# wing02/MyLdpcCppApi

Measured on AMD Instinct MI355X. Metric: decoded Mbit/s (info bits), DVB-S2 N=64800 rate-1/2, 50 iters, higher is better.
Workload: dtype f32; 1 GPU; DVB-S2-profile (64800,32400) rate-1/2 (seeded IRA table with the standard's structure, E=226799), batch 4096 frames per GPU, 50 iterations, sum-product fp32 (probability domain), all-zero codeword + AWGN sigma=0.95 (no frame converges), early termination on, inputs resident in HBM; global_batch=4096, frames_per_gpu=4096, algo=sp, frames_per_launch=4096, parallelism=frames sharded over 1 GPU(s), all-gather of decoded bytes, frames_converged=0

## Files before the change

### myldpccppapi_amd/csrc/flood_kernels.hpp

```cpp
#pragma once

#include <hip/hip_runtime.h>
#include <stdint.h>

#include "ldpc_expf.h"

namespace ldpc {

constexpr int kAlgoSP = 0;
constexpr int kAlgoMS = 1;
constexpr int kAlgoMSC = 2;
constexpr int kCompactCapacity = 512;
constexpr int kLastCapacity = 64;
constexpr int kBlock = 256;
constexpr int kWavesPerBlock = 4;
constexpr int kMaxUnrolledDegree = 16;
constexpr int kMaxUnrolledCheckDegreeMS = 32;

#ifndef LDPC_NT_LOAD
#define LDPC_NT_LOAD 1
#endif
#ifndef LDPC_NT_STORE
#define LDPC_NT_STORE 1
#endif
typedef float vf2 __attribute__((ext_vector_type(2)));
typedef float vf4 __attribute__((ext_vector_type(4)));

template <typename T> __device__ __forceinline__ T ld_stream(const T *p)
{
#if LDPC_NT_LOAD
    return __builtin_nontemporal_load(p);
#else
    return *p;
#endif
}
template <typename T> __device__ __forceinline__ void st_stream(T *p, T v)
{
#if LDPC_NT_STORE
    __builtin_nontemporal_store(v, p);
#else
    *p = v;
#endif
}

template <int V> __device__ __forceinline__ void vload(float (&d)[V], const float *p);
template <> __device__ __forceinline__ void vload<1>(float (&d)[1], const float *p) { d[0] = ld_stream(p); }
template <> __device__ __forceinline__ void vload<2>(float (&d)[2], const float *p)
{
    const vf2 t = ld_stream(reinterpret_cast<const vf2 *>(p));
    d[0] = t.x; d[1] = t.y;
}
template <> __device__ __forceinline__ void vload<4>(float (&d)[4], const float *p)
{
    const vf4 t = ld_stream(reinterpret_cast<const vf4 *>(p));
    d[0] = t.x; d[1] = t.y; d[2] = t.z; d[3] = t.w;
}
template <int V> __device__ __forceinline__ void vstore(float *p, const float (&s)[V]);
template <> __device__ __forceinline__ void vstore<1>(float *p, const float (&s)[1]) { st_stream(p, s[0]); }
template <> __device__ __forceinline__ void vstore<2>(float *p, const float (&s)[2])
{
    vf2 t; t.x = s[0]; t.y = s[1];
    st_stream(reinterpret_cast<vf2 *>(p), t);
}
template <> __device__ __forceinline__ void vstore<4>(float *p, const float (&s)[4])
{
    vf4 t; t.x = s[0]; t.y = s[1]; t.z = s[2]; t.w = s[3];
    st_stream(reinterpret_cast<vf4 *>(p), t);
}

typedef _Float16 hf;
typedef _Float16 vh2 __attribute__((ext_vector_type(2)));
typedef _Float16 vh4 __attribute__((ext_vector_type(4)));

template <int V> __device__ __forceinline__ void vload(float (&d)[V], const hf *p);
template <> __device__ __forceinline__ void vload<1>(float (&d)[1], const hf *p) { d[0] = (float)ld_stream(p); }
template <> __device__ __forceinline__ void vload<2>(float (&d)[2], const hf *p)
{
    const vh2 t = ld_stream(reinterpret_cast<const vh2 *>(p));
    d[0] = (float)t.x; d[1] = (float)t.y;
}
template <> __device__ __forceinline__ void vload<4>(float (&d)[4], const hf *p)
{
    const vh4 t = ld_stream(reinterpret_cast<const vh4 *>(p));
    d[0] = (float)t.x; d[1] = (float)t.y; d[2] = (float)t.z; d[3] = (float)t.w;
}
template <int V> __device__ __forceinline__ void vstore(hf *p, const float (&s)[V]);
template <> __device__ __forceinline__ void vstore<1>(hf *p, const float (&s)[1]) { st_stream(p, (hf)s[0]); }
template <> __device__ __forceinline__ void vstore<2>(hf *p, const float (&s)[2])
{
    vh2 t; t.x = (hf)s[0]; t.y = (hf)s[1];
    st_stream(reinterpret_cast<vh2 *>(p), t);
}
template <> __device__ __forceinline__ void vstore<4>(hf *p, const float (&s)[4])
{
    vh4 t; t.x = (hf)s[0]; t.y = (hf)s[1]; t.z = (hf)s[2]; t.w = (hf)s[3];
    st_stream(reinterpret_cast<vh4 *>(p), t);
}

__device__ __forceinline__ int wave_id_in_block()
{
    return __builtin_amdgcn_readfirstlane((int)(threadIdx.x >> 6));
}

template <int V> __device__ __forceinline__ bool tile_finished(const uint64_t *done, int tile)
{
    bool all = true;
#pragma unroll
    for (int v = 0; v < V; ++v) all = all && (done[(size_t)tile * V + v] == ~0ull);
    return all;
}

struct TailRef {
    const int32_t *state;
    int32_t base_tile;
    int32_t n_tiles;
};

template <int V> __device__ __forceinline__ int tile_select(const TailRef &t, const uint64_t *done, int row)
{
    int tile = row;
    if (t.state && __builtin_amdgcn_readfirstlane(t.state[0])) {
        if (row >= t.n_tiles) return -1;
        tile = t.base_tile + row;
    }
    return tile_finished<V>(done, tile) ? -1 : tile;
}


struct CheckArgs {
    const void *__restrict__ Q;
    void *__restrict__ R;
    const int32_t *__restrict__ cls_e0;
    const uint64_t *__restrict__ done;
    int64_t E;
    int32_t n_rows;
    int32_t rows_per_wave;
    int32_t degree;
    float ms_scale = 1.0f;
    TailRef tail;
    int32_t tiles_first = 0;
    float ms_offset = 0.0f;
    const void *__restrict__ first_chan = nullptr;
    const int32_t *__restrict__ edge_col = nullptr;
    int32_t N = 0;
    const int32_t *__restrict__ qpos = nullptr;
};

template <int D> __device__ __forceinline__ void row_slots(const int32_t *__restrict__ qpos, int e0, int lane, int (&slot)[D])
{
    static_assert(D <= 64, "one lane per edge");
    const int mine = qpos[e0 + (lane < D ? lane : D - 1)];
#pragma unroll
    for (int k = 0; k < D; ++k) slot[k] = __builtin_amdgcn_readlane(mine, k);
}
__device__ __forceinline__ int edge_slot(const int32_t *__restrict__ qpos, int e)
{
    return __builtin_amdgcn_readfirstlane(qpos[e]);
}

struct GridPos { int row, block; };
__device__ __forceinline__ GridPos grid_pos(int tiles_first)
{
    return tiles_first ? GridPos{(int)blockIdx.x, (int)blockIdx.y} : GridPos{(int)blockIdx.y, (int)blockIdx.x};
}

template <int D, int V>
__device__ __forceinline__ void check_sp(const float (&x)[D][V], float (&out)[D][V])
{
#pragma unroll
    for (int v = 0; v < V; ++v) {
        if (D == 1) { out[0][v] = 1.0f; continue; }
        {
            float p = x[1][v];
#pragma unroll
            for (int j = 2; j < D; ++j) p *= x[j][v];
            out[0][v] = p;
        }
        float pre = x[0][v];
#pragma unroll
        for (int k = 1; k < D; ++k) {
            float p = pre;
#pragma unroll
            for (int j = k + 1; j < D; ++j) p *= x[j][v];
            out[k][v] = p;
            pre *= x[k][v];
        }
    }
}

struct MsCorr {
    float scale, offset;
};
template <typename T> __device__ __forceinline__ float ms_corr(float m, const MsCorr &c)
{
    const float r = fmaxf(m - c.offset, 0.0f) * c.scale;
    return sizeof(T) == 2 ? (float)(hf)r : r;
}

template <int D, int V, bool CORR = false, typename T = float>
__device__ __forceinline__ void check_ms(const float (&x)[D][V], float (&out)[D][V], MsCorr c = MsCorr{1.0f, 0.0f})
{
#pragma unroll
    for (int v = 0; v < V; ++v) {
        float m1 = 1000.0f, m2 = 1000.0f;
        int idx = -1;
        unsigned par = 0;
#pragma unroll
        for (int j = 0; j < D; ++j) {
            const float a = __builtin_fabsf(x[j][v]);
            par ^= (x[j][v] < 0.0f) ? 1u : 0u;
            if (a < m1) { m2 = m1; m1 = a; idx = j; }
            else if (a < m2) { m2 = a; }
        }
        if (CORR) { m1 = ms_corr<T>(m1, c); m2 = ms_corr<T>(m2, c); }
#pragma unroll
        for (int k = 0; k < D; ++k) {
            const float b = (k == idx) ? m2 : m1;
            const unsigned s = par ^ ((x[k][v] < 0.0f) ? 1u : 0u);
            out[k][v] = s ? -b : b;
        }
    }
}

__device__ __forceinline__ MsCorr ms_corr_of(const CheckArgs &a) { return MsCorr{a.ms_scale, a.ms_offset}; }

template <int ALGO, int D, int V, int W, typename T>
__global__ __launch_bounds__(kBlock) void check_kernel(const CheckArgs a)
{
    constexpr size_t F = 64 * V;
    constexpr int SUB = V / W;
    const int lane = threadIdx.x & 63;
    const GridPos gp = grid_pos(a.tiles_first);
    const int tile = tile_select<V>(a.tail, a.done, gp.row);
    if (tile < 0) return;
    const int wave = gp.block * kWavesPerBlock + wave_id_in_block();
    const int sub = wave % SUB;
    const int r_begin = (wave / SUB) * a.rows_per_wave;
    const int r_end = min(r_begin + a.rows_per_wave, a.n_rows);
    const unsigned lane_off = (unsigned)sub * 64 * W + (unsigned)lane * W;
    const T *Qu = static_cast<const T *>(a.Q) + (size_t)tile * (size_t)a.E * F;
    T *Rt = static_cast<T *>(a.R) + (size_t)tile * (size_t)a.E * F + lane_off;

    const T *Ct = (ALGO != kAlgoSP && a.first_chan)
                      ? static_cast<const T *>(a.first_chan) + (size_t)tile * (size_t)a.N * F + lane_off : nullptr;
    for (int r = r_begin; r < r_end; ++r) {
        const int e0 = a.cls_e0[r];
        float x[D][W], out[D][W];
        if (ALGO != kAlgoSP && Ct) {
#pragma unroll
            for (int k = 0; k < D; ++k) vload<W>(x[k], Ct + (size_t)a.edge_col[e0 + k] * F);
        } else {
            int sl[D];
            row_slots<D>(a.qpos, e0, lane, sl);
#pragma unroll
            for (int k = 0; k < D; ++k) vload<W>(x[k], Qu + (size_t)sl[k] * F + lane_off);
        }
        if (ALGO == kAlgoSP) check_sp<D, W>(x, out); else if (ALGO == kAlgoMS) check_ms<D, W>(x, out); else check_ms<D, W, true, T>(x, out, ms_corr_of(a));
#pragma unroll
        for (int k = 0; k < D; ++k) vstore<W>(Rt + (size_t)(e0 + k) * F, out[k]);
    }
}

template <int ALGO, int V, typename T>
__device__ __forceinline__ void check_row_generic(const T *Qu, unsigned lane_off, T *Rt, int e0, int D,
                                                  const int32_t *__restrict__ qpos, const MsCorr &c)
{
    constexpr size_t F = 64 * V;
    if (ALGO != kAlgoSP) {
        float m1[V], m2[V];
        int idx[V];
        unsigned par[V];
#pragma unroll
        for (int v = 0; v < V; ++v) { m1[v] = 1000.0f; m2[v] = 1000.0f; idx[v] = -1; par[v] = 0; }
        for (int j = 0; j < D; ++j) {
            float xj[V];
            vload<V>(xj, Qu + (size_t)edge_slot(qpos, e0 + j) * F + lane_off);
#pragma unroll
            for (int v = 0; v < V; ++v) {
                const float m = __builtin_fabsf(xj[v]);
                par[v] ^= (xj[v] < 0.0f) ? 1u : 0u;
                if (m < m1[v]) { m2[v] = m1[v]; m1[v] = m; idx[v] = j; }
                else if (m < m2[v]) { m2[v] = m; }
            }
        }
        if (ALGO == kAlgoMSC) {
#pragma unroll
            for (int v = 0; v < V; ++v) { m1[v] = ms_corr<T>(m1[v], c); m2[v] = ms_corr<T>(m2[v], c); }
        }
        for (int k = 0; k < D; ++k) {
            float xk[V], o[V];
            vload<V>(xk, Qu + (size_t)edge_slot(qpos, e0 + k) * F + lane_off);
#pragma unroll
            for (int v = 0; v < V; ++v) {
                const float b = (k == idx[v]) ? m2[v] : m1[v];
                const unsigned sg = par[v] ^ ((xk[v] < 0.0f) ? 1u : 0u);
                o[v] = sg ? -b : b;
            }
            vstore<V>(Rt + (size_t)(e0 + k) * F, o);
        }
        return;
    }
    for (int k = 0; k < D; ++k) {
        float o[V];
        float p[V];
#pragma unroll
        for (int v = 0; v < V; ++v) p[v] = 1.0f;
        for (int j = 0; j < D; ++j) {
            if (j == k) continue;
            float xj[V];
            vload<V>(xj, Qu + (size_t)edge_slot(qpos, e0 + j) * F + lane_off);
#pragma unroll
            for (int v = 0; v < V; ++v) p[v] *= xj[v];
        }
#pragma unroll
        for (int v = 0; v < V; ++v) o[v] = p[v];
        vstore<V>(Rt + (size_t)(e0 + k) * F, o);
    }
}

template <int ALGO, int V, typename T>
__global__ __launch_bounds__(kBlock) void check_kernel_generic(const CheckArgs a)
{
    constexpr size_t F = 64 * V;
    const int lane = threadIdx.x & 63;
    const GridPos gp = grid_pos(a.tiles_first);
    const int tile = tile_select<V>(a.tail, a.done, gp.row);
    if (tile < 0) return;
    const int wave = gp.block * kWavesPerBlock + wave_id_in_block();
    const int r_begin = wave * a.rows_per_wave;
    const int r_end = min(r_begin + a.rows_per_wave, a.n_rows);
    const T *Qu = static_cast<const T *>(a.Q) + (size_t)tile * (size_t)a.E * F;
    T *Rt = static_cast<T *>(a.R) + (size_t)tile * (size_t)a.E * F + (size_t)lane * V;
    for (int r = r_begin; r < r_end; ++r) check_row_generic<ALGO, V, T>(Qu, (unsigned)lane * V, Rt, a.cls_e0[r], a.degree, a.qpos, ms_corr_of(a));
}

struct GroupClass {
    int32_t block_begin;
    int32_t degree;
    int32_t count;
    int32_t pad;
    const int32_t *ids;
    const int32_t *edges;
    int64_t q_base;
};

template <int ALGO, int D, int V, int W, typename T>
__device__ __forceinline__ void check_rows(const T *Qu, unsigned lane_off, T *Rt, const int32_t *__restrict__ e0s, int r_begin, int r_end,
                                           const T *Ct, const int32_t *__restrict__ edge_col,
                                           const int32_t *__restrict__ qpos, const MsCorr &c)
{
    const int lane = threadIdx.x & 63;
    constexpr size_t F = 64 * V;
    for (int r = r_begin; r < r_end; ++r) {
        const int e0 = e0s[r];
        float x[D][W], out[D][W];
        if (ALGO != kAlgoSP && Ct) {
#pragma unroll
            for (int k = 0; k < D; ++k) vload<W>(x[k], Ct + (size_t)edge_col[e0 + k] * F);
        } else {
            int sl[D];
            row_slots<D>(qpos, e0, lane, sl);
#pragma unroll
            for (int k = 0; k < D; ++k) vload<W>(x[k], Qu + (size_t)sl[k] * F + lane_off);
        }
        if (ALGO == kAlgoSP) check_sp<D, W>(x, out); else if (ALGO == kAlgoMS) check_ms<D, W>(x, out); else check_ms<D, W, true, T>(x, out, c);
#pragma unroll
        for (int k = 0; k < D; ++k) vstore<W>(Rt + (size_t)(e0 + k) * F, out[k]);
    }
}

template <int ALGO, int V, typename T, int D, int DLO, int W = 1> struct CheckDispatch {
    static __device__ __forceinline__ void run(int deg, const T *Qu, unsigned lane_off, T *Rt, const int32_t *e0s, int rb, int re,
                                               const T *Ct, const int32_t *edge_col, const int32_t *qpos, const MsCorr &c)
    {
        if (deg == D) check_rows<ALGO, D, V, W, T>(Qu, lane_off, Rt, e0s, rb, re, Ct, edge_col, qpos, c);
        else CheckDispatch<ALGO, V, T, D - 1, DLO, W>::run(deg, Qu, lane_off, Rt, e0s, rb, re, Ct, edge_col, qpos, c);
    }
};
template <int ALGO, int V, typename T, int DLO, int W> struct CheckDispatch<ALGO, V, T, DLO, DLO, W> {
    static __device__ __forceinline__ void run(int, const T *Qu, unsigned lane_off, T *Rt, const int32_t *e0s, int rb, int re,
                                               const T *Ct, const int32_t *edge_col, const int32_t *qpos, const MsCorr &c)
    {
        check_rows<ALGO, DLO, V, W, T>(Qu, lane_off, Rt, e0s, rb, re, Ct, edge_col, qpos, c);
    }
};

template <int ALGO, int V, typename T, int DLO, int DHI, int W = 1>
__global__ __launch_bounds__(kBlock) void check_group_kernel(const CheckArgs a, const GroupClass *__restrict__ cls, int n_classes)
{
    constexpr size_t F = 64 * V;
    constexpr int SUB = V / W;
    const int lane = threadIdx.x & 63;
    const GridPos gp = grid_pos(a.tiles_first);
    const int tile = tile_select<V>(a.tail, a.done, gp.row);
    if (tile < 0) return;
    int c = 0;
    while (c + 1 < n_classes && gp.block >= cls[c + 1].block_begin) ++c;
    const int wave = (gp.block - cls[c].block_begin) * kWavesPerBlock + wave_id_in_block();
    const int sub = wave % SUB;
    const int r_begin = (wave / SUB) * a.rows_per_wave;
    const int r_end = min(r_begin + a.rows_per_wave, cls[c].count);
    const unsigned lane_off = (unsigned)sub * 64 * W + (unsigned)lane * W;
    const T *Qu = static_cast<const T *>(a.Q) + (size_t)tile * (size_t)a.E * F;
    T *Rt = static_cast<T *>(a.R) + (size_t)tile * (size_t)a.E * F + lane_off;
    const T *Ct = (ALGO != kAlgoSP && a.first_chan)
                      ? static_cast<const T *>(a.first_chan) + (size_t)tile * (size_t)a.N * F + lane_off : nullptr;
    CheckDispatch<ALGO, V, T, DHI, DLO, W>::run(cls[c].degree, Qu, lane_off, Rt, cls[c].ids, r_begin, r_end, Ct, a.edge_col, a.qpos, ms_corr_of(a));
}

struct SyndromeArgs {
    const int32_t *__restrict__ row_ptr;
    const int32_t *__restrict__ edge_col;
    const uint64_t *__restrict__ hard;
    uint64_t *__restrict__ fail;
    const uint64_t *__restrict__ done;
    int32_t M, N;
    int32_t tiles;
    int32_t row_blocks;
    TailRef tail;
};

template <int V> __global__ __launch_bounds__(kBlock) void syndrome_kernel(const SyndromeArgs a)
{
    int tile, rb;
    if (a.tiles > 0) {
        const int xcd = blockIdx.x & 7, j = blockIdx.x >> 3;
        tile = xcd + 8 * (j / a.row_blocks);
        rb = j % a.row_blocks;
        if (tile >= a.tiles) return;
    } else {
        tile = blockIdx.y;
        rb = blockIdx.x;
    }
    tile = tile_select<V>(a.tail, a.done, tile);
    if (tile < 0) return;
    const int m = rb * kBlock + threadIdx.x;
    const uint64_t *hard_t = a.hard + (size_t)tile * (size_t)a.N * V;
    uint64_t s[V];
#pragma unroll
    for (int v = 0; v < V; ++v) s[v] = 0;
    if (m < a.M) {
        for (int p = a.row_ptr[m]; p < a.row_ptr[m + 1]; ++p) {
            const int c = a.edge_col[p];
#pragma unroll
            for (int v = 0; v < V; ++v) s[v] ^= hard_t[(size_t)c * V + v];
        }
    }
    __shared__ uint64_t part[kWavesPerBlock][V];
#pragma unroll
    for (int v = 0; v < V; ++v) {
        uint64_t x = s[v];
#pragma unroll
        for (int off = 32; off >= 1; off >>= 1) {
            const uint32_t lo = __shfl_xor((uint32_t)x, off);
            const uint32_t hi = __shfl_xor((uint32_t)(x >> 32), off);
            x |= ((uint64_t)hi << 32) | lo;
        }
        if ((threadIdx.x & 63) == 0) part[threadIdx.x >> 6][v] = x;
    }
    __syncthreads();
    if (threadIdx.x < V) {
        uint64_t x = 0;
#pragma unroll
        for (int w = 0; w < kWavesPerBlock; ++w) x |= part[w][threadIdx.x];
        unsigned long long *dst = reinterpret_cast<unsigned long long *>(&a.fail[(size_t)tile * V + threadIdx.x]);
        const uint64_t seen = __hip_atomic_load(dst, __ATOMIC_RELAXED, __HIP_MEMORY_SCOPE_AGENT);
        if (x & ~seen) atomicOr(dst, (unsigned long long)x);
    }
}


struct VarArgs {
    const void *__restrict__ R;
    void *__restrict__ Q;
    const void *__restrict__ chan;
    uint64_t *hard;
    const uint64_t *__restrict__ done;
    const int32_t *__restrict__ cls_col;
    const int32_t *__restrict__ cls_edge;
    int64_t E;
    int32_t N;
    int32_t n_cols;
    int32_t cols_per_wave;
    int32_t write_q;
    int32_t degree;
    TailRef tail;
    int32_t tiles_first = 0;
    int64_t q_base = -1;
};

template <int D, int V>
__device__ __forceinline__ void var_sp(const float (&t)[V], const float (&d)[D][V],
                                       float (&outq)[D][V], float (&full0)[V], float (&full1)[V])
{
#pragma unroll
    for (int v = 0; v < V; ++v) {
        const float den = 1.0f + t[v];
        float pre0 = t[v] / den;
        float pre1 = 1.0f / den;
        float r0[D], r1[D];
#pragma unroll
        for (int k = 0; k < D; ++k) {
            r0[k] = (1.0f + d[k][v]) * 0.5f;
            r1[k] = (1.0f - d[k][v]) * 0.5f;
        }
#pragma unroll
        for (int k = 0; k < D; ++k) {
            float t0 = pre0, t1 = pre1;
#pragma unroll
            for (int j = k + 1; j < D; ++j) { t0 *= r0[j]; t1 *= r1[j]; }
            const float s = t0 + t1;
            const float q0 = t0 / s;
            const float q1 = t1 / s;
            outq[k][v] = q0 - q1;
            pre0 *= r0[k];
            pre1 *= r1[k];
        }
        full0[v] = pre0;
        full1[v] = pre1;
    }
}

struct LinkArgs {
    const int32_t *__restrict__ link_col;
    const int32_t *__restrict__ link_pos;
    const void *__restrict__ chan;
    void *Qw;
    uint64_t *hard;
    int32_t N;
    int32_t write_q;
    int32_t store_all;
    const int32_t *__restrict__ extra_e0;
    const int32_t *__restrict__ extra_deg;
    int32_t n_extra;
    int32_t link_blocks;
    int32_t n_big, small_rows;
};

__host__ __device__ inline void link_chunk_rows(int c, int rows_per_wave, int n_big, int small_rows, int n_rows,
                                               int *rb, int *re)
{
    int b, e;
    if (c < n_big) { b = c * rows_per_wave; e = b + rows_per_wave; }
    else { b = n_big * rows_per_wave + (c - n_big) * small_rows; e = b + small_rows; }
    *rb = b < n_rows ? b : n_rows;
    *re = e < n_rows ? e : n_rows;
}
__host__ __device__ inline int link_chunk_count(int rows_per_wave, int n_big, int small_rows, int n_rows)
{
    const int rest = n_rows - n_big * rows_per_wave;
    return n_big + (rest > 0 ? (rest + small_rows - 1) / small_rows : 0);
}

template <int ALGO, int V, typename T>
__device__ __forceinline__ void link_extra_rows(const CheckArgs &a, const LinkArgs &g, int tile, int block)
{
    constexpr size_t F = 64 * V;
    const int lane = threadIdx.x & 63;
    const int w = (block - g.link_blocks) * kWavesPerBlock + wave_id_in_block();
    if (w >= g.n_extra) return;
    const T *Qu = static_cast<const T *>(a.Q) + (size_t)tile * (size_t)a.E * F;
    T *Rt = static_cast<T *>(a.R) + (size_t)tile * (size_t)a.E * F + (size_t)lane * V;
    check_row_generic<ALGO, V, T>(Qu, (unsigned)lane * V, Rt, g.extra_e0[w], g.extra_deg[w], a.qpos, ms_corr_of(a));
}

#ifdef LDPC_LINK_WIDE_WAVES
#define LDPC_LINK_WIDE_ATTR __attribute__((amdgpu_waves_per_eu(LDPC_LINK_WIDE_WAVES, LDPC_LINK_WIDE_WAVES)))
#else
#define LDPC_LINK_WIDE_ATTR
#endif
template <int ALGO, int D, int V, typename T>
__global__ __launch_bounds__(kBlock) LDPC_LINK_WIDE_ATTR void check_link_kernel(const CheckArgs a, const LinkArgs g)
{
    constexpr size_t F = 64 * V;
    const int lane = threadIdx.x & 63;
    const GridPos gp = grid_pos(a.tiles_first);
    const int tile = tile_select<V>(a.tail, a.done, gp.row);
    if (tile < 0) return;
    if (gp.block >= g.link_blocks) { link_extra_rows<ALGO, V, T>(a, g, tile, gp.block); return; }
    const int wave = gp.block * kWavesPerBlock + wave_id_in_block();
    int r_begin, r_end;
    link_chunk_rows(wave, a.rows_per_wave, g.n_big, g.small_rows, a.n_rows, &r_begin, &r_end);
    const size_t lane_off = (size_t)lane * V;
    const unsigned lane_q = (unsigned)lane * V;
    const T *Qt = static_cast<const T *>(a.Q) + (size_t)tile * (size_t)a.E * F;
    T *Qwt = static_cast<T *>(g.Qw) + (size_t)tile * (size_t)a.E * F;
    T *Rt = static_cast<T *>(a.R) + (size_t)tile * (size_t)a.E * F + lane_off;
    const T *chan_t = static_cast<const T *>(g.chan) + (size_t)tile * (size_t)g.N * F + lane_off;
    uint64_t *hard_t = g.hard + (size_t)tile * (size_t)g.N * V;
    uint64_t frozen[V];
#pragma unroll
    for (int v = 0; v < V; ++v) frozen[v] = a.done[(size_t)tile * V + v];

    int pend_col = -1, pend_edge = 0, pend_kb = 0;
    float pend_r[V];
#pragma unroll
    for (int v = 0; v < V; ++v) pend_r[v] = 0.0f;

    float x[D][V];
    int qc[D], qn[D];
#pragma unroll
    for (int k = 0; k < D; ++k) qc[k] = qn[k] = 0;
    if (r_begin < r_end) {
        row_slots<D>(a.qpos, a.cls_e0[r_begin], lane, qc);
#pragma unroll
        for (int k = 0; k < D; ++k) vload<V>(x[k], Qt + (size_t)qc[k] * F + lane_q);
    }
    for (int r = r_begin; r < r_end; ++r) {
        const int e0 = a.cls_e0[r];
        const int next_col = (r + 1 < r_end) ? g.link_col[r] : -1;
        const int pos = g.link_pos[r];
        const int ka = next_col >= 0 ? (pos & 255) : -1;
        const int kb = pend_col >= 0 ? pend_kb : -1;
        if (r + 1 < r_end) row_slots<D>(a.qpos, a.cls_e0[r + 1], lane, qn);
        float ch[V];
        uint64_t old_w[V];
        if (pend_col >= 0) {
            vload<V>(ch, chan_t + (size_t)pend_col * F);
#pragma unroll
            for (int v = 0; v < V; ++v) old_w[v] = hard_t[(size_t)pend_col * V + v];
        }
        float out[D][V];
        if (ALGO == kAlgoSP) check_sp<D, V>(x, out); else if (ALGO == kAlgoMS) check_ms<D, V>(x, out); else check_ms<D, V, true, T>(x, out, ms_corr_of(a));
        if (r + 1 < r_end) {
#pragma unroll
            for (int k = 0; k < D; ++k) vload<V>(x[k], Qt + (size_t)qn[k] * F + lane_q);
        }
#pragma unroll
        for (int k = 0; k < D; ++k)
            if ((k != ka && k != kb) || g.store_all) vstore<V>(Rt + (size_t)(e0 + k) * F, out[k]);

        if (pend_col >= 0) {
            float rr[2][V], q[2][V];
#pragma unroll
            for (int v = 0; v < V; ++v) {
                rr[0][v] = pend_r[v];
                float t = out[0][v];
#pragma unroll
                for (int k = 1; k < D; ++k) t = (k == kb) ? out[k][v] : t;
                rr[1][v] = t;
            }
            uint64_t new_w[V];
            if (ALGO == kAlgoSP) {
                float f0[V], f1[V];
                var_sp<2, V>(ch, rr, q, f0, f1);
#pragma unroll
                for (int v = 0; v < V; ++v) {
                    const bool oldb = (old_w[v] >> lane) & 1ull;
                    const bool b = (f0[v] > f1[v]) ? false : ((f0[v] < f1[v]) ? true : oldb);
                    new_w[v] = __ballot(b);
                }
            } else {
#pragma unroll
                for (int v = 0; v < V; ++v) {
                    float p = ch[v];
                    p += rr[0][v];
                    p += rr[1][v];
                    q[0][v] = p - rr[0][v];
                    q[1][v] = p - rr[1][v];
                    new_w[v] = __ballot(!(p > 0.0f));
                }
            }
            if (lane == 0) {
#pragma unroll
                for (int v = 0; v < V; ++v)
                    hard_t[(size_t)pend_col * V + v] = (old_w[v] & frozen[v]) | (new_w[v] & ~frozen[v]);
            }
            if (g.write_q) {
                int qw1 = qc[0];
#pragma unroll
                for (int k = 1; k < D; ++k) qw1 = (k == kb) ? qc[k] : qw1;
                vstore<V>(Qwt + (size_t)pend_edge * F + lane_q, q[0]);
                vstore<V>(Qwt + (size_t)qw1 * F + lane_q, q[1]);
            }
        }
        pend_col = next_col;
        if (next_col >= 0) {
            pend_edge = qc[0];
#pragma unroll
            for (int k = 1; k < D; ++k) pend_edge = (k == ka) ? qc[k] : pend_edge;
            pend_kb = (pos >> 8) & 255;
#pragma unroll
            for (int v = 0; v < V; ++v) {
                float t = out[0][v];
#pragma unroll
                for (int k = 1; k < D; ++k) t = (k == ka) ? out[k][v] : t;
                pend_r[v] = t;
            }
        }
#pragma unroll
        for (int k = 0; k < D; ++k) qc[k] = qn[k];
    }
}

template <int V> __device__ __forceinline__ uint64_t compress_stride(uint64_t x)
{
    if (V == 1) return x;
    if (V == 2) {
        x &= 0x5555555555555555ull;
        x = (x | (x >> 1)) & 0x3333333333333333ull;
        x = (x | (x >> 2)) & 0x0f0f0f0f0f0f0f0full;
        x = (x | (x >> 4)) & 0x00ff00ff00ff00ffull;
        x = (x | (x >> 8)) & 0x0000ffff0000ffffull;
        x = (x | (x >> 16)) & 0x00000000ffffffffull;
        return x;
    }
    x &= 0x1111111111111111ull;
    x = (x | (x >> 3)) & 0x0303030303030303ull;
    x = (x | (x >> 6)) & 0x000f000f000f000full;
    x = (x | (x >> 12)) & 0x000000ff000000ffull;
    x = (x | (x >> 24)) & 0x000000000000ffffull;
    return x;
}

template <int ALGO, int D, int V, typename T, int W = 1>
__global__ __launch_bounds__(kBlock) void check_link_narrow_kernel(const CheckArgs a, const LinkArgs g)
{
    constexpr size_t F = 64 * V;
    constexpr int SUBS = V / W;
    constexpr int FB = 64 / SUBS;
    const int lane = threadIdx.x & 63;
    const GridPos gp = grid_pos(a.tiles_first);
    const int tile = tile_select<V>(a.tail, a.done, gp.row);
    if (tile < 0) return;
    if (gp.block >= g.link_blocks) { link_extra_rows<ALGO, V, T>(a, g, tile, gp.block); return; }
    const int wave = gp.block * kWavesPerBlock + wave_id_in_block();
    const int sub = wave % SUBS;
    int r_begin, r_end;
    link_chunk_rows(wave / SUBS, a.rows_per_wave, g.n_big, g.small_rows, a.n_rows, &r_begin, &r_end);
    const size_t lane_off = (size_t)sub * 64 * W + (size_t)lane * W;
    const unsigned lane_q = (unsigned)lane_off;
    const T *Qt = static_cast<const T *>(a.Q) + (size_t)tile * (size_t)a.E * F;
    T *Qwt = static_cast<T *>(g.Qw) + (size_t)tile * (size_t)a.E * F;
    T *Rt = static_cast<T *>(a.R) + (size_t)tile * (size_t)a.E * F + lane_off;
    const T *chan_t = static_cast<const T *>(g.chan) + (size_t)tile * (size_t)g.N * F + lane_off;
    uint8_t *hard_b = reinterpret_cast<uint8_t *>(g.hard + (size_t)tile * (size_t)g.N * V) + (size_t)sub * (FB / 8);
    const uint64_t frozen_field = (a.done[(size_t)tile * V + (lane < V ? lane : 0)] >> (sub * FB)) &
                                  (FB == 64 ? ~0ull : ((1ull << (FB & 63)) - 1ull));

    auto load_field = [&](int col, int word) -> uint64_t {
        const uint8_t *p = hard_b + ((size_t)col * V + word) * 8;
        if (FB == 64) return *reinterpret_cast<const uint64_t *>(p);
        if (FB == 32) return *reinterpret_cast<const uint32_t *>(p);
        return *reinterpret_cast<const uint16_t *>(p);
    };

    int pend_col = -1, pend_edge = 0, pend_kb = 0;
    float pend_r[W];
#pragma unroll
    for (int w = 0; w < W; ++w) pend_r[w] = 0.0f;
    float x[D][W];
    int qc[D], qn[D];
#pragma unroll
    for (int k = 0; k < D; ++k) qc[k] = qn[k] = 0;
    if (r_begin < r_end) {
        row_slots<D>(a.qpos, a.cls_e0[r_begin], lane, qc);
#pragma unroll
        for (int k = 0; k < D; ++k) vload<W>(x[k], Qt + (size_t)qc[k] * F + lane_q);
    }
    for (int r = r_begin; r < r_end; ++r) {
        const int e0 = a.cls_e0[r];
        const int next_col = (r + 1 < r_end) ? g.link_col[r] : -1;
        const int pos = g.link_pos[r];
        const int ka = next_col >= 0 ? (pos & 255) : -1;
        const int kb = pend_col >= 0 ? pend_kb : -1;
        if (r + 1 < r_end) row_slots<D>(a.qpos, a.cls_e0[r + 1], lane, qn);
        float ch[W];
        uint64_t old_mine[W];
#pragma unroll
        for (int w = 0; w < W; ++w) { ch[w] = 0.0f; old_mine[w] = 0; }
        if (pend_col >= 0) {
            vload<W>(ch, chan_t + (size_t)pend_col * F);
#pragma unroll
            for (int w = 0; w < W; ++w) old_mine[w] = load_field(pend_col, (W * lane + w) % V);
        }
        float out[D][W];
        if (ALGO == kAlgoSP) check_sp<D, W>(x, out); else if (ALGO == kAlgoMS) check_ms<D, W>(x, out); else check_ms<D, W, true, T>(x, out, ms_corr_of(a));
        if (r + 1 < r_end) {
#pragma unroll
            for (int k = 0; k < D; ++k) vload<W>(x[k], Qt + (size_t)qn[k] * F + lane_q);
        }
#pragma unroll
        for (int k = 0; k < D; ++k)
            if ((k != ka && k != kb) || g.store_all) vstore<W>(Rt + (size_t)(e0 + k) * F, out[k]);

        if (pend_col >= 0) {
            float rr[2][W], q[2][W];
#pragma unroll
            for (int w = 0; w < W; ++w) {
                rr[0][w] = pend_r[w];
                float t = out[0][w];
#pragma unroll
                for (int k = 1; k < D; ++k) t = (k == kb) ? out[k][w] : t;
                rr[1][w] = t;
            }
            uint64_t ballot[W];
            if (ALGO == kAlgoSP) {
                float f0[W], f1[W];
                var_sp<2, W>(ch, rr, q, f0, f1);
#pragma unroll
                for (int w = 0; w < W; ++w) {
                    const bool oldb = (old_mine[w] >> ((W * lane + w) / V)) & 1ull;
                    const bool bit = (f0[w] > f1[w]) ? false : ((f0[w] < f1[w]) ? true : oldb);
                    ballot[w] = __ballot(bit);
                }
            } else {
#pragma unroll
                for (int w = 0; w < W; ++w) {
                    float p = ch[w];
                    p += rr[0][w];
                    p += rr[1][w];
                    q[0][w] = p - rr[0][w];
                    q[1][w] = p - rr[1][w];
                    ballot[w] = __ballot(!(p > 0.0f));
                }
            }
            if (lane < V) {
                uint64_t bw = ballot[0];
#pragma unroll
                for (int w = 1; w < W; ++w) bw = (lane % W == w) ? ballot[w] : bw;
                const uint64_t nf = compress_stride<SUBS>(bw >> (lane / W));
                const uint64_t of = load_field(pend_col, lane);
                const uint64_t res = (of & frozen_field) | (nf & ~frozen_field);
                uint8_t *p = hard_b + ((size_t)pend_col * V + lane) * 8;
                if (FB == 64) *reinterpret_cast<uint64_t *>(p) = res;
                else if (FB == 32) *reinterpret_cast<uint32_t *>(p) = (uint32_t)res;
                else *reinterpret_cast<uint16_t *>(p) = (uint16_t)res;
            }
            if (g.write_q) {
                int qw1 = qc[0];
#pragma unroll
                for (int k = 1; k < D; ++k) qw1 = (k == kb) ? qc[k] : qw1;
                vstore<W>(Qwt + (size_t)pend_edge * F + lane_q, q[0]);
                vstore<W>(Qwt + (size_t)qw1 * F + lane_q, q[1]);
            }
        }
        pend_col = next_col;
        if (next_col >= 0) {
            pend_edge = qc[0];
#pragma unroll
            for (int k = 1; k < D; ++k) pend_edge = (k == ka) ? qc[k] : pend_edge;
            pend_kb = (pos >> 8) & 255;
#pragma unroll
            for (int w = 0; w < W; ++w) {
                float t = out[0][w];
#pragma unroll
                for (int k = 1; k < D; ++k) t = (k == ka) ? out[k][w] : t;
                pend_r[w] = t;
            }
        }
#pragma unroll
        for (int k = 0; k < D; ++k) qc[k] = qn[k];
    }
}

template <int ALGO, int D, int V, typename T>
__global__ __launch_bounds__(kBlock) void check_link_narrow2_kernel(const CheckArgs a, const LinkArgs g)
{
    constexpr size_t F = 64 * V;
    constexpr int FB = 64 / V;
    const int lane = threadIdx.x & 63;
    const GridPos gp = grid_pos(a.tiles_first);
    const int tile = tile_select<V>(a.tail, a.done, gp.row);
    if (tile < 0) return;
    if (gp.block >= g.link_blocks) { link_extra_rows<ALGO, V, T>(a, g, tile, gp.block); return; }
    const int wave = gp.block * kWavesPerBlock + wave_id_in_block();
    const int sub = wave % V;
    int r_begin, r_end;
    link_chunk_rows(wave / V, a.rows_per_wave, g.n_big, g.small_rows, a.n_rows, &r_begin, &r_end);
    const size_t lane_off = (size_t)sub * 64 + lane;
    const T *Qt = static_cast<const T *>(a.Q) + (size_t)tile * (size_t)a.E * F + lane_off;
    T *Qwt = static_cast<T *>(g.Qw) + (size_t)tile * (size_t)a.E * F + lane_off;
    T *Rt = static_cast<T *>(a.R) + (size_t)tile * (size_t)a.E * F + lane_off;
    const T *chan_t = static_cast<const T *>(g.chan) + (size_t)tile * (size_t)g.N * F + lane_off;
    const int my_word = lane % V, my_bit = lane / V;
    uint8_t *hard_b = reinterpret_cast<uint8_t *>(g.hard + (size_t)tile * (size_t)g.N * V) + (size_t)sub * (FB / 8);
    const uint64_t frozen_field = (a.done[(size_t)tile * V + (lane < V ? lane : 0)] >> (sub * FB)) &
                                  (FB == 64 ? ~0ull : ((1ull << FB) - 1ull));

    auto load_field = [&](int col, int word) -> uint64_t {
        const uint8_t *p = hard_b + ((size_t)col * V + word) * 8;
        if (V == 1) return *reinterpret_cast<const uint64_t *>(p);
        if (V == 2) return *reinterpret_cast<const uint32_t *>(p);
        return *reinterpret_cast<const uint16_t *>(p);
    };

    int pend_col = -1, pend_edge = 0, pend_kb = 0;
    float pend_r = 0.0f;
    float b0[D], b1[D], b2[D];
    auto load_row = [&](float (&dst)[D], int r) {
        const int e = a.cls_e0[r];
#pragma unroll
        for (int k = 0; k < D; ++k) { float t[1]; vload<1>(t, Qt + (size_t)edge_slot(a.qpos, e + k) * F); dst[k] = t[0]; }
    };
    if (r_begin < r_end) load_row(b0, r_begin);
    if (r_begin + 1 < r_end) load_row(b1, r_begin + 1);
    auto step = [&](int r, float (&x)[D], float (&pre)[D]) {
        const int e0 = a.cls_e0[r];
        const int next_col = (r + 1 < r_end) ? g.link_col[r] : -1;
        const int pos = g.link_pos[r];
        const int ka = next_col >= 0 ? (pos & 255) : -1;
        const int kb = pend_col >= 0 ? pend_kb : -1;
        float ch[1] = {0.0f};
        uint64_t old_mine = 0;
        if (pend_col >= 0) {
            vload<1>(ch, chan_t + (size_t)pend_col * F);
            old_mine = load_field(pend_col, my_word);
        }
        if (r + 2 < r_end) load_row(pre, r + 2);
        float xx[D][1], out[D][1];
#pragma unroll
        for (int k = 0; k < D; ++k) xx[k][0] = x[k];
        if (ALGO == kAlgoSP) check_sp<D, 1>(xx, out); else if (ALGO == kAlgoMS) check_ms<D, 1>(xx, out); else check_ms<D, 1, true, T>(xx, out, ms_corr_of(a));
#pragma unroll
        for (int k = 0; k < D; ++k)
            if ((k != ka && k != kb) || g.store_all) vstore<1>(Rt + (size_t)(e0 + k) * F, out[k]);

        if (pend_col >= 0) {
            float rr[2][1], q[2][1];
            rr[0][0] = pend_r;
            float t = out[0][0];
#pragma unroll
            for (int k = 1; k < D; ++k) t = (k == kb) ? out[k][0] : t;
            rr[1][0] = t;
            bool bit;
            if (ALGO == kAlgoSP) {
                float f0[1], f1[1];
                var_sp<2, 1>(ch, rr, q, f0, f1);
                const bool oldb = (old_mine >> my_bit) & 1ull;
                bit = (f0[0] > f1[0]) ? false : ((f0[0] < f1[0]) ? true : oldb);
            } else {
                float p = ch[0];
                p += rr[0][0];
                p += rr[1][0];
                q[0][0] = p - rr[0][0];
                q[1][0] = p - rr[1][0];
                bit = !(p > 0.0f);
            }
            const uint64_t ballot = __ballot(bit);
            if (lane < V) {
                const uint64_t nf = compress_stride<V>(ballot >> lane);
                const uint64_t of = load_field(pend_col, lane);
                const uint64_t res = (of & frozen_field) | (nf & ~frozen_field);
                uint8_t *p = hard_b + ((size_t)pend_col * V + lane) * 8;
                if (V == 1) *reinterpret_cast<uint64_t *>(p) = res;
                else if (V == 2) *reinterpret_cast<uint32_t *>(p) = (uint32_t)res;
                else *reinterpret_cast<uint16_t *>(p) = (uint16_t)res;
            }
            if (g.write_q) {
                vstore<1>(Qwt + (size_t)edge_slot(a.qpos, pend_edge) * F, q[0]);
                vstore<1>(Qwt + (size_t)edge_slot(a.qpos, e0 + kb) * F, q[1]);
            }
        }
        pend_col = next_col;
        if (next_col >= 0) {
            pend_edge = e0 + ka;
            pend_kb = (pos >> 8) & 255;
            float t = out[0][0];
#pragma unroll
            for (int k = 1; k < D; ++k) t = (k == ka) ? out[k][0] : t;
            pend_r = t;
        }
    };
    for (int r = r_begin; r < r_end; r += 3) {
        step(r, b0, b2);
        if (r + 1 < r_end) step(r + 1, b1, b0);
        if (r + 2 < r_end) step(r + 2, b2, b1);
    }
}

template <int ALGO, int D, int V, typename T>
__device__ __forceinline__ void var_columns(const T *Rt, T *Qt, const T *chan_t, uint64_t *hard_t, const uint64_t (&frozen)[V],
                                            const int32_t *__restrict__ cls_col, const int32_t *__restrict__ cls_edge,
                                            int c_begin, int c_end, int write_q, int lane, int64_t q_base, int n_cls)
{
    constexpr size_t F = 64 * V;
    for (int ci = c_begin; ci < c_end; ++ci) {
        const int n = cls_col[ci];
        int e[D];
#pragma unroll
        for (int k = 0; k < D; ++k) e[k] = cls_edge[(size_t)ci * D + k];
        float ch[V], r[D][V], q[D][V];
        vload<V>(ch, chan_t + (size_t)n * F);
#pragma unroll
        for (int k = 0; k < D; ++k) vload<V>(r[k], Rt + (size_t)e[k] * F);
        uint64_t old_w[V], new_w[V];
#pragma unroll
        for (int v = 0; v < V; ++v) old_w[v] = hard_t[(size_t)n * V + v];

        if (ALGO == kAlgoSP) {
            float f0[V], f1[V];
            var_sp<D, V>(ch, r, q, f0, f1);
#pragma unroll
            for (int v = 0; v < V; ++v) {
                const bool oldb = (old_w[v] >> lane) & 1ull;
                const bool b = (f0[v] > f1[v]) ? false : ((f0[v] < f1[v]) ? true : oldb);
                new_w[v] = __ballot(b);
            }
        } else {
#pragma unroll
            for (int v = 0; v < V; ++v) {
                float p = ch[v];
#pragma unroll
                for (int k = 0; k < D; ++k) p += r[k][v];
#pragma unroll
                for (int k = 0; k < D; ++k) q[k][v] = p - r[k][v];
                new_w[v] = __ballot(!(p > 0.0f));
            }
        }
        if (lane == 0) {
#pragma unroll
            for (int v = 0; v < V; ++v)
                hard_t[(size_t)n * V + v] = (old_w[v] & frozen[v]) | (new_w[v] & ~frozen[v]);
        }
        if (write_q) {
            if (q_base >= 0) {
                T *Qc = Qt + ((size_t)q_base + (size_t)ci) * F;
#pragma unroll
                for (int k = 0; k < D; ++k) vstore<V>(Qc + (size_t)k * (size_t)n_cls * F, q[k]);
            } else {
#pragma unroll
                for (int k = 0; k < D; ++k) vstore<V>(Qt + (size_t)e[k] * F, q[k]);
            }
        }
    }
}

#ifdef LDPC_VAR_WAVES
#define LDPC_VAR_ATTR __attribute__((amdgpu_waves_per_eu(LDPC_VAR_WAVES, LDPC_VAR_WAVES)))
#else
#define LDPC_VAR_ATTR
#endif
template <int ALGO, int D, int V, typename T>
__global__ __launch_bounds__(kBlock) LDPC_VAR_ATTR void var_kernel(const VarArgs a)
{
    constexpr size_t F = 64 * V;
    const int lane = threadIdx.x & 63;
    const GridPos gp = grid_pos(a.tiles_first);
    const int tile = tile_select<V>(a.tail, a.done, gp.row);
    if (tile < 0) return;
    const int wave = gp.block * kWavesPerBlock + wave_id_in_block();
    const int c_begin = wave * a.cols_per_wave;
    const int c_end = min(c_begin + a.cols_per_wave, a.n_cols);
    const T *Rt = static_cast<const T *>(a.R) + (size_t)tile * (size_t)a.E * F + (size_t)lane * V;
    T *Qt = static_cast<T *>(a.Q) + (size_t)tile * (size_t)a.E * F + (size_t)lane * V;
    const T *chan_t = static_cast<const T *>(a.chan) + (size_t)tile * (size_t)a.N * F + (size_t)lane * V;
    uint64_t *hard_t = a.hard + (size_t)tile * (size_t)a.N * V;
    uint64_t frozen[V];
#pragma unroll
    for (int v = 0; v < V; ++v) frozen[v] = a.done[(size_t)tile * V + v];
    var_columns<ALGO, D, V, T>(Rt, Qt, chan_t, hard_t, frozen, a.cls_col, a.cls_edge, c_begin, c_end, a.write_q, lane, a.q_base, a.n_cols);
}

template <int ALGO, int V, typename T, int D, int DLO> struct VarDispatch {
    static __device__ __forceinline__ void run(int deg, const T *Rt, T *Qt, const T *chan_t, uint64_t *hard_t,
                                               const uint64_t (&frozen)[V], const int32_t *col, const int32_t *edge,
                                               int cb, int ce, int write_q, int lane, int64_t q_base, int n_cls)
    {
        if (deg == D) var_columns<ALGO, D, V, T>(Rt, Qt, chan_t, hard_t, frozen, col, edge, cb, ce, write_q, lane, q_base, n_cls);
        else VarDispatch<ALGO, V, T, D - 1, DLO>::run(deg, Rt, Qt, chan_t, hard_t, frozen, col, edge, cb, ce, write_q, lane, q_base, n_cls);
    }
};
template <int ALGO, int V, typename T, int DLO> struct VarDispatch<ALGO, V, T, DLO, DLO> {
    static __device__ __forceinline__ void run(int, const T *Rt, T *Qt, const T *chan_t, uint64_t *hard_t,
                                               const uint64_t (&frozen)[V], const int32_t *col, const int32_t *edge,
                                               int cb, int ce, int write_q, int lane, int64_t q_base, int n_cls)
    {
        var_columns<ALGO, DLO, V, T>(Rt, Qt, chan_t, hard_t, frozen, col, edge, cb, ce, write_q, lane, q_base, n_cls);
    }
};

template <int ALGO, int V, typename T, int DLO, int DHI>
__global__ __launch_bounds__(kBlock) void var_group_kernel(const VarArgs a, const GroupClass *__restrict__ cls, int n_classes)
{
    constexpr size_t F = 64 * V;
    const int lane = threadIdx.x & 63;
    const GridPos gp = grid_pos(a.tiles_first);
    const int tile = tile_select<V>(a.tail, a.done, gp.row);
    if (tile < 0) return;
    int c = 0;
    while (c + 1 < n_classes && gp.block >= cls[c + 1].block_begin) ++c;
    const int wave = (gp.block - cls[c].block_begin) * kWavesPerBlock + wave_id_in_block();
    const int c_begin = wave * a.cols_per_wave;
    const int c_end = min(c_begin + a.cols_per_wave, cls[c].count);
    const T *Rt = static_cast<const T *>(a.R) + (size_t)tile * (size_t)a.E * F + (size_t)lane * V;
    T *Qt = static_cast<T *>(a.Q) + (size_t)tile * (size_t)a.E * F + (size_t)lane * V;
    const T *chan_t = static_cast<const T *>(a.chan) + (size_t)tile * (size_t)a.N * F + (size_t)lane * V;
    uint64_t *hard_t = a.hard + (size_t)tile * (size_t)a.N * V;
    uint64_t frozen[V];
#pragma unroll
    for (int v = 0; v < V; ++v) frozen[v] = a.done[(size_t)tile * V + v];
    VarDispatch<ALGO, V, T, DHI, DLO>::run(cls[c].degree, Rt, Qt, chan_t, hard_t, frozen, cls[c].ids, cls[c].edges,
                                           c_begin, c_end, a.write_q, lane, cls[c].q_base, cls[c].count);
}

template <int ALGO, int V, typename T>
__global__ __launch_bounds__(kBlock) void var_kernel_generic(const VarArgs a)
{
    constexpr size_t F = 64 * V;
    const int lane = threadIdx.x & 63;
    const GridPos gp = grid_pos(a.tiles_first);
    const int tile = tile_select<V>(a.tail, a.done, gp.row);
    if (tile < 0) return;
    const int wave = gp.block * kWavesPerBlock + wave_id_in_block();
    const int c_begin = wave * a.cols_per_wave;
    const int c_end = min(c_begin + a.cols_per_wave, a.n_cols);
    const int D = a.degree;
    const T *Rt = static_cast<const T *>(a.R) + (size_t)tile * (size_t)a.E * F + (size_t)lane * V;
    T *Qt = static_cast<T *>(a.Q) + (size_t)tile * (size_t)a.E * F + (size_t)lane * V;
    const T *chan_t = static_cast<const T *>(a.chan) + (size_t)tile * (size_t)a.N * F + (size_t)lane * V;
    uint64_t *hard_t = a.hard + (size_t)tile * (size_t)a.N * V;
    uint64_t frozen[V];
#pragma unroll
    for (int v = 0; v < V; ++v) frozen[v] = a.done[(size_t)tile * V + v];

    for (int ci = c_begin; ci < c_end; ++ci) {
        const int n = a.cls_col[ci];
        const int32_t *e = a.cls_edge + (size_t)ci * D;
        auto qs = [&](int k) -> size_t { return a.q_base >= 0 ? (size_t)a.q_base + (size_t)k * a.n_cols + ci : (size_t)e[k]; };
        float ch[V];
        vload<V>(ch, chan_t + (size_t)n * F);
        uint64_t old_w[V], new_w[V];
#pragma unroll
        for (int v = 0; v < V; ++v) old_w[v] = hard_t[(size_t)n * V + v];
        if (ALGO == kAlgoSP) {
            float p0[V], p1[V];
#pragma unroll
            for (int v = 0; v < V; ++v) {
                const float den = 1.0f + ch[v];
                p0[v] = ch[v] / den;
                p1[v] = 1.0f / den;
            }
            for (int k = 0; k <= D; ++k) {
                float t0[V], t1[V];
#pragma unroll
                for (int v = 0; v < V; ++v) { t0[v] = p0[v]; t1[v] = p1[v]; }
                for (int j = 0; j < D; ++j) {
                    if (j == k) continue;
                    float dj[V];
                    vload<V>(dj, Rt + (size_t)e[j] * F);
#pragma unroll
                    for (int v = 0; v < V; ++v) {
                        t0[v] *= (1.0f + dj[v]) * 0.5f;
                        t1[v] *= (1.0f - dj[v]) * 0.5f;
                    }
                }
                if (k < D) {
                    if (a.write_q) {
                        float o[V];
#pragma unroll
                        for (int v = 0; v < V; ++v) {
                            const float s = t0[v] + t1[v];
                            o[v] = t0[v] / s - t1[v] / s;
                        }
                        vstore<V>(Qt + qs(k) * F, o);
                    }
                } else {
#pragma unroll
                    for (int v = 0; v < V; ++v) {
                        const bool oldb = (old_w[v] >> lane) & 1ull;
                        const bool b = (t0[v] > t1[v]) ? false : ((t0[v] < t1[v]) ? true : oldb);
                        new_w[v] = __ballot(b);
                    }
                }
            }
        } else {
            float p[V];
#pragma unroll
            for (int v = 0; v < V; ++v) p[v] = ch[v];
            for (int j = 0; j < D; ++j) {
                float rj[V];
                vload<V>(rj, Rt + (size_t)e[j] * F);
#pragma unroll
                for (int v = 0; v < V; ++v) p[v] += rj[v];
            }
#pragma unroll
            for (int v = 0; v < V; ++v) new_w[v] = __ballot(!(p[v] > 0.0f));
            if (a.write_q) {
                for (int j = 0; j < D; ++j) {
                    float rj[V], o[V];
                    vload<V>(rj, Rt + (size_t)e[j] * F);
#pragma unroll
                    for (int v = 0; v < V; ++v) o[v] = p[v] - rj[v];
                    vstore<V>(Qt + qs(j) * F, o);
                }
            }
        }
        if (lane == 0) {
#pragma unroll
            for (int v = 0; v < V; ++v)
                hard_t[(size_t)n * V + v] = (old_w[v] & frozen[v]) | (new_w[v] & ~frozen[v]);
        }
    }
}


struct InitArgs {
    const float *__restrict__ llr;
    void *__restrict__ chan;
    void *__restrict__ Q;
    uint64_t *__restrict__ hard;
    const int32_t *__restrict__ col_ptr;
    const int32_t *__restrict__ col_edge;
    int64_t E;
    int64_t frames;
    int32_t N;
    float llr_scale;
};

constexpr int kInitCols = 32;

template <int ALGO, int V, typename T>
__global__ __launch_bounds__(kBlock) void init_kernel(const InitArgs a)
{
    constexpr int F = 64 * V;
// ... 563 lines not shown
```

### myldpccppapi_amd/csrc/flood_tables.hpp

```cpp
#pragma once

#include "flood_kernels.hpp"

namespace ldpc {

using CheckFn = void (*)(const CheckArgs);
using VarFn = void (*)(const VarArgs);
using LinkFn = void (*)(const CheckArgs, const LinkArgs);
using CheckGroupFn = void (*)(const CheckArgs, const GroupClass *, int);
using VarGroupFn = void (*)(const VarArgs, const GroupClass *, int);
using InitFn = void (*)(const InitArgs);

constexpr int kVarBuckets = 3, kCheckBuckets = 4;
constexpr int kVarBucketLo[kVarBuckets] = {1, 5, 9}, kVarBucketHi[kVarBuckets] = {4, 8, 16};
constexpr int kCheckBucketLo[kCheckBuckets] = {1, 9, 17, 25}, kCheckBucketHi[kCheckBuckets] = {8, 16, 24, 32};

struct FloodFns {
    CheckFn check[kMaxUnrolledCheckDegreeMS + 1] = {};
    CheckFn check_wide[kMaxUnrolledCheckDegreeMS + 1] = {};
    LinkFn link[kMaxUnrolledDegree + 1] = {};
    LinkFn link_narrow[kMaxUnrolledDegree + 1] = {};
    LinkFn link_deep[kMaxUnrolledDegree + 1] = {};
    LinkFn link_half[kMaxUnrolledDegree + 1] = {};
    VarFn var[kMaxUnrolledDegree + 1] = {};
    CheckGroupFn check_group[kCheckBuckets] = {};
    int check_group_width = 1;
    VarGroupFn var_group[kVarBuckets] = {};
    InitFn init = nullptr;
    int max_check_unrolled = kMaxUnrolledDegree;
};

void fill_flood_sp(int V, FloodFns *f);
void fill_flood_ms(int V, FloodFns *f);
void fill_flood_ms16(int V, FloodFns *f);
void fill_flood_msc(int V, FloodFns *f);
void fill_flood_msc16(int V, FloodFns *f);

}
```

### myldpccppapi_amd/csrc/flood_tables_impl.hpp

```cpp
#pragma once

#include "flood_tables.hpp"

namespace ldpc {
namespace tables {

template <int ALGO, int V, typename T, int D> struct FloodTable {
    static void fill(CheckFn *c, CheckFn *cw, VarFn *v)
    {
        c[D] = check_kernel<ALGO, D, V, 1, T>;
        cw[D] = check_kernel<ALGO, D, V, V, T>;
        v[D] = var_kernel<ALGO, D, V, T>;
        FloodTable<ALGO, V, T, D - 1>::fill(c, cw, v);
    }
};
template <int ALGO, int V, typename T> struct FloodTable<ALGO, V, T, 0> {
    static void fill(CheckFn *c, CheckFn *cw, VarFn *v)
    {
        c[0] = cw[0] = check_kernel_generic<ALGO, V, T>;
        v[0] = var_kernel_generic<ALGO, V, T>;
    }
};

template <int ALGO, int V, typename T, int D> struct CheckTableMS {
    static void fill(CheckFn *c, CheckFn *cw)
    {
        c[D] = cw[D] = check_kernel<ALGO, D, V, 1, T>;
        CheckTableMS<ALGO, V, T, D - 1>::fill(c, cw);
    }
};
template <int ALGO, int V, typename T> struct CheckTableMS<ALGO, V, T, kMaxUnrolledDegree> {
    static void fill(CheckFn *, CheckFn *) {}
};

template <int ALGO, int V, typename T, int D> struct LinkHalf {
    static LinkFn get() { return nullptr; }
};
template <int ALGO, typename T, int D> struct LinkHalf<ALGO, 4, T, D> {
    static LinkFn get() { return check_link_narrow_kernel<ALGO, D, 4, T, 2>; }
};
template <int ALGO, int V, typename T, int D> struct LinkTable {
    static void fill(LinkFn *t, LinkFn *tn, LinkFn *td, LinkFn *th)
    {
        t[D] = check_link_kernel<ALGO, D, V, T>;
        tn[D] = check_link_narrow_kernel<ALGO, D, V, T>;
        td[D] = check_link_narrow2_kernel<ALGO, D, V, T>;
        th[D] = LinkHalf<ALGO, V, T, D>::get();
        LinkTable<ALGO, V, T, D - 1>::fill(t, tn, td, th);
    }
};
template <int ALGO, int V, typename T> struct LinkTable<ALGO, V, T, 1> {
    static void fill(LinkFn *, LinkFn *, LinkFn *, LinkFn *) {}
};

template <int ALGO, int V, typename T> void fill_v(FloodFns *f)
{
    constexpr int DM = kMaxUnrolledDegree;
    FloodTable<ALGO, V, T, DM>::fill(f->check, f->check_wide, f->var);
    LinkTable<ALGO, V, T, DM>::fill(f->link, f->link_narrow, f->link_deep, f->link_half);
    constexpr int GW = (sizeof(T) == 2 && V == 4) ? 2 : 1;
    f->check_group_width = GW;
    f->check_group[0] = check_group_kernel<ALGO, V, T, 1, 8, GW>;
    f->check_group[1] = check_group_kernel<ALGO, V, T, 9, 16, GW>;
    f->check_group[2] = f->check_group[3] = nullptr;
    f->var_group[0] = var_group_kernel<ALGO, V, T, 1, 4>;
    f->var_group[1] = var_group_kernel<ALGO, V, T, 5, 8>;
    f->var_group[2] = var_group_kernel<ALGO, V, T, 9, 16>;
    f->init = init_kernel<ALGO, V, T>;
    f->max_check_unrolled = DM;
    if (ALGO != kAlgoSP) {
        CheckTableMS<ALGO, V, T, kMaxUnrolledCheckDegreeMS>::fill(f->check, f->check_wide);
        f->check_group[2] = check_group_kernel<ALGO, V, T, 17, 24, GW>;
        f->check_group[3] = check_group_kernel<ALGO, V, T, 25, 32, GW>;
        f->max_check_unrolled = kMaxUnrolledCheckDegreeMS;
    }
}

template <int ALGO, typename T> void fill(int V, FloodFns *f)
{
    *f = FloodFns();
    if (V == 1) fill_v<ALGO, 1, T>(f);
    else if (V == 2) fill_v<ALGO, 2, T>(f);
    else fill_v<ALGO, 4, T>(f);
}

}
}
```

### myldpccppapi_amd/csrc/ldpc_hip.hip

```cpp
#include <hip/hip_runtime.h>

#include <algorithm>
#include <chrono>
#include <cstdarg>
#include <cstdio>
#include <cstdlib>
#include <cstring>
#include <map>
#include <memory>
#include <new>
#include <string>
#include <thread>
#include <vector>

#include "../../include/ldpc_hip.h"
#include "flood_kernels.hpp"
#include "flood_tables.hpp"
#include "layered_kernels.hpp"
#include "fused_kernels.hpp"
#include "ldsp_kernels.hpp"
#include "engines.hpp"
#include "channel_kernels.hpp"
#include "tune.hpp"
#include "host_stage.hpp"
#include "graph.hpp"

#ifndef LDPC_IDLE_FAT
#define LDPC_IDLE_FAT 8
#endif

namespace {

thread_local std::string g_err;

int fail(int code, const char *fmt, ...)
{
    char buf[512];
    va_list ap;
    va_start(ap, fmt);
    vsnprintf(buf, sizeof buf, fmt, ap);
    va_end(ap);
    g_err = buf;
    return code;
}

#define HIP_TRY(expr)                                                                  \
    do {                                                                               \
        hipError_t e_ = (expr);                                                        \
        if (e_ != hipSuccess)                                                          \
            return fail(LDPC_ERR_HIP, "%s failed: %s (%s:%d)", #expr, hipGetErrorString(e_), \
                        __FILE__, __LINE__);                                           \
    } while (0)

template <typename T> struct DevBuf {
    T *p = nullptr;
    size_t n = 0;
    DevBuf() = default;
    DevBuf(const DevBuf &) = delete;
    DevBuf &operator=(const DevBuf &) = delete;
    DevBuf(DevBuf &&o) noexcept : p(o.p), n(o.n) { o.p = nullptr; o.n = 0; }
    DevBuf &operator=(DevBuf &&o) noexcept
    {
        if (this != &o) { release(); p = o.p; n = o.n; o.p = nullptr; o.n = 0; }
        return *this;
    }
    hipError_t alloc(size_t count)
    {
        release();
        n = count;
        if (!count) return hipSuccess;
        return hipMalloc((void **)&p, count * sizeof(T));
    }
    hipError_t upload(const std::vector<T> &h)
    {
        hipError_t e = alloc(h.size());
        if (e != hipSuccess || h.empty()) return e;
        return hipMemcpy(p, h.data(), h.size() * sizeof(T), hipMemcpyHostToDevice);
    }
    void release()
    {
        if (p) (void)hipFree(p);
        p = nullptr;
        n = 0;
    }
    ~DevBuf() { release(); }
};

}



int ldpc::set_error(int code, const char *fmt, ...)
{
    char buf[512];
    va_list ap;
    va_start(ap, fmt);
    vsnprintf(buf, sizeof buf, fmt, ap);
    va_end(ap);
    g_err = buf;
    return code;
}


namespace {

using ldpc::CheckFn;
using ldpc::VarFn;
using ldpc::LinkFn;
using ldpc::CheckGroupFn;
using ldpc::VarGroupFn;
using ldpc::InitFn;
using ldpc::kVarBuckets;
using ldpc::kCheckBuckets;
using ldpc::kVarBucketLo;
using ldpc::kVarBucketHi;
using ldpc::kCheckBucketLo;
using ldpc::kCheckBucketHi;

struct RowClass {
    int degree = 0;
    int count = 0;
    DevBuf<int32_t> e0;
    std::vector<int32_t> h_e0;
    DevBuf<int32_t> link_col, link_pos;
    int linked = 0;
    int n_big = 0, small_rows = 1;
};
struct ColClass {
    int degree = 0;
    int count = 0;
    DevBuf<int32_t> col, edge;
    int64_t q_base = -1;
};

struct ClassGroup {
    int bucket = 0, lo = 0, hi = 0;
    int blocks = 0;
    int blocks_fat = 0;
    std::vector<int> members;
    DevBuf<ldpc::GroupClass> table, table_fat;
};

constexpr int kIdleFat = LDPC_IDLE_FAT;

struct TimedSpan {
    hipEvent_t a, b;
    int kind;
    int degree;
    int64_t bytes;
    int64_t moved;
    int lo;
};

}

struct ldpc_decoder {
    ldpc_decoder_config cfg{};
    int32_t M = 0, N = 0;
    int64_t E = 0;
    int V = 1, F = 64, T = 0;
    std::vector<int32_t> h_col_ptr, h_col_edge, h_rows, h_cols;

    DevBuf<int32_t> row_ptr, edge_col, col_ptr, col_edge;
    DevBuf<int32_t> qpos, col_qedge;
    std::vector<int32_t> h_qpos;
    DevBuf<uint8_t> chan, Q, R;
    int msg_size = 4;
    InitFn init_fn = nullptr;
    DevBuf<uint64_t> hard, failw, done;
    DevBuf<int32_t> iters, active;
    std::vector<RowClass> row_classes;
    std::vector<ColClass> col_classes;
    std::vector<ClassGroup> check_groups, var_groups;
    std::vector<int> check_solo, var_solo;
    CheckGroupFn check_group_fn[kCheckBuckets] = {};
    int check_group_width = 1;
    VarGroupFn var_group_fn[kVarBuckets] = {};
    DevBuf<int32_t> extra_e0, extra_deg;
    int n_extra = 0;
    int64_t extra_edges = 0;
    CheckFn check_fn[ldpc::kMaxUnrolledCheckDegreeMS + 1] = {};
    CheckFn check_fn_wide[ldpc::kMaxUnrolledCheckDegreeMS + 1] = {};
    int max_check_unrolled = ldpc::kMaxUnrolledDegree;
    LinkFn link_fn[ldpc::kMaxUnrolledDegree + 1] = {};
    LinkFn link_narrow_fn[ldpc::kMaxUnrolledDegree + 1] = {};
    LinkFn link_deep_fn[ldpc::kMaxUnrolledDegree + 1] = {};
    LinkFn link_half_fn[ldpc::kMaxUnrolledDegree + 1] = {};
    int tune_link_deep = 0;
    ldpc::Tune tune;
    int tune_link_narrow = 1;
    bool link_calibrated = false;
    float link_cal_ms[3] = {0, 0, 0};
    int place_candidates = 0, place_kept = 0;
    float place_ms[16] = {};
    int link_rpw = 16;
    int tune_link_guided = 0;
    int tune_tiles_first = 0;
    int cus = 256;
    VarFn var_fn[ldpc::kMaxUnrolledDegree + 1] = {};

    ldpc::LayeredPlan layered;
    ldpc::FusedPlan fused;
    bool use_fused = false;
    ldpc::LdspPlan ldsp;
    bool use_ldsp = false;
    bool ms_corr = false;
    float ms_scale = 1.0f, ms_offset = 0.0f;

    hipStream_t stream = nullptr, copy_stream = nullptr;
    struct HostSlot {
        DevBuf<float> llr;
        DevBuf<uint8_t> out;
        DevBuf<int32_t> iters;
        uint8_t *h_out = nullptr;
        int32_t *h_iters = nullptr;
        uint8_t *h_head = nullptr;
        hipEvent_t h2d_done = nullptr, all_done = nullptr;
        bool busy = false;
        int64_t off = 0, n = 0, dst = 0, copy_bytes = 0;
        int32_t *h_sum = nullptr;
        int g_iterations = 0, g_tiles = 0, g_children = 0, g_child_f[3] = {0, 0, 0};
    } slot[3];
    struct CallCounts { bool valid = false; int32_t iterations = 0, batch_time = 0; int64_t frames = 0, converged = 0, frame_rounds = 0; } call;
    bool suppress_poll = false;
    int32_t *h_active = nullptr;
    struct RingChunk { uint8_t *h = nullptr; hipEvent_t ev = nullptr; bool used = false; };
    std::vector<RingChunk> ring;
    size_t ring_next = 0;
    std::unique_ptr<ldpc::Worker> stager;
    std::vector<std::unique_ptr<ldpc::Worker>> copy_helpers;
    std::vector<ldpc::Job> copy_jobs;
    ldpc::Job stage_job[3];
    bool stage_pending[3] = {false, false, false};
    std::vector<void *> locked_blocks, stuck_blocks;
    ldpc_decoder *child = nullptr;
    DevBuf<int32_t> cmap;
    DevBuf<int32_t> cinv;
    DevBuf<unsigned long long> cmoved;
    int child_capacity = ldpc::kCompactCapacity;
    int compact_threshold = ldpc::kCompactCapacity;
    bool is_child = false;
    bool tail_enabled = false;
    int TO = 0, TA = 0;
    DevBuf<int32_t> tail_state, tail_map, running;
    int32_t *h_summary = nullptr;
    hipEvent_t ev_summary = nullptr;
    bool summary_pending = false;
    int idle_after = 0;

    bool timing = false;
    int timing_every = 0;
    int64_t timing_calls = 0;
    std::vector<TimedSpan> spans;
    size_t spans_used = 0;
    hipEvent_t ev_begin = nullptr, ev_end = nullptr;
    hipStream_t last_stream = nullptr;
    bool have_last = false;
    int32_t tap_iter = 0;
    int tune_rpw = 0, tune_cpw = 0;
    int tune_syn_xcd = 1;
    int tune_check_wide = 0;
    int32_t last_iterations = 0;
    int64_t last_frames = 0;
    DevBuf<int32_t> summary;
    ldpc_decoder *handed_to = nullptr;
    bool first_round_from_chan = false;
    int32_t last_tiles = 0;

    std::vector<ldpc_decoder *> shards;
    std::vector<std::unique_ptr<ldpc::Worker>> shard_workers;

    ~ldpc_decoder()
    {
        for (auto &w : shard_workers) w->stop();
        if (stager) stager->stop();
        for (auto &w : copy_helpers) w->stop();
        for (ldpc_decoder *sh : shards) (void)ldpc_decoder_destroy(sh);
        for (auto &s : spans) { (void)hipEventDestroy(s.a); (void)hipEventDestroy(s.b); }
        if (ev_begin) (void)hipEventDestroy(ev_begin);
        if (ev_end) (void)hipEventDestroy(ev_end);
        if (h_active) (void)hipHostFree(h_active);
        for (auto &rc : ring) {
            if (rc.h) (void)hipHostFree(rc.h);
            if (rc.ev) (void)hipEventDestroy(rc.ev);
        }
        if (h_summary) (void)hipHostFree(h_summary);
        if (ev_summary) (void)hipEventDestroy(ev_summary);
        for (auto &sl : slot) {
            if (sl.h_out) (void)hipHostFree(sl.h_out);
            if (sl.h_iters) (void)hipHostFree(sl.h_iters);
            if (sl.h_head) (void)hipHostFree(sl.h_head);
            if (sl.h_sum) (void)hipHostFree(sl.h_sum);
            if (sl.h2d_done) (void)hipEventDestroy(sl.h2d_done);
            if (sl.all_done) (void)hipEventDestroy(sl.all_done);
        }
        if (copy_stream) (void)hipStreamDestroy(copy_stream);
        if (stream) (void)hipStreamDestroy(stream);
        delete child;
    }
};

namespace {

template <bool NT>
__global__ __launch_bounds__(256) void hbm_probe_copy_kernel(const ldpc::vf4 *__restrict__ src, ldpc::vf4 *__restrict__ dst, size_t n4)
{
    const size_t stride = (size_t)gridDim.x * 256 * 4;
    for (size_t i = (size_t)blockIdx.x * 256 * 4 + threadIdx.x; i < n4; i += stride) {
        ldpc::vf4 v[4];
#pragma unroll
        for (int k = 0; k < 4; ++k)
            if (i + (size_t)k * 256 < n4) v[k] = NT ? __builtin_nontemporal_load(&src[i + (size_t)k * 256]) : src[i + (size_t)k * 256];
#pragma unroll
        for (int k = 0; k < 4; ++k)
            if (i + (size_t)k * 256 < n4) {
                if (NT) __builtin_nontemporal_store(v[k], &dst[i + (size_t)k * 256]);
                else dst[i + (size_t)k * 256] = v[k];
            }
    }
}

template <int V>
__global__ void summary_kernel(const int32_t *iters, const uint64_t *done, const uint64_t *fail,
                               int64_t frames, int32_t freeze, int32_t *summary)
{
    constexpr int F = 64 * V;
    const int64_t f = (int64_t)blockIdx.x * blockDim.x + threadIdx.x;
    if (f >= frames) return;
    const int64_t tile = f / F;
    const int fi = (int)(f % F);
    const int l = fi / V, v = fi % V;
    atomicMax(&summary[0], iters[f]);
    const uint64_t ok = freeze ? done[tile * V + v] : ~fail[tile * V + v];
    if ((ok >> l) & 1ull) atomicAdd(&summary[1], 1);
}

int pick_frames_per_lane(const ldpc_decoder_config &cfg, int32_t max_row_deg, int32_t max_col_deg)
{
    if (cfg.frames_per_lane) return cfg.frames_per_lane;
    int deg = cfg.algo == LDPC_ALGO_LAYERED ? max_row_deg : max_col_deg;
    if (cfg.algo == LDPC_ALGO_MS) deg = (deg + 1) / 2;
    if (cfg.max_batch >= 1024 && deg <= 8) return 4;
    if (cfg.max_batch >= 256 && deg <= ldpc::kMaxUnrolledDegree) return 2;
    return 1;
}

hipError_t span_begin(ldpc_decoder *d, hipStream_t s, int kind, int degree = 0, int64_t bytes = 0, int64_t moved = -1,
                      int lo = 0)
{
    if (!d->timing) return hipSuccess;
    if (d->spans_used == d->spans.size()) {
        TimedSpan t{};
        hipError_t e = hipEventCreate(&t.a);
        if (e != hipSuccess) return e;
        e = hipEventCreate(&t.b);
        if (e != hipSuccess) return e;
        d->spans.push_back(t);
    }
    d->spans[d->spans_used].kind = kind;
    d->spans[d->spans_used].degree = degree;
    d->spans[d->spans_used].bytes = bytes;
    d->spans[d->spans_used].moved = moved < 0 ? bytes : moved;
    d->spans[d->spans_used].lo = lo;
    return hipEventRecord(d->spans[d->spans_used].a, s);
}

hipError_t span_end(ldpc_decoder *d, hipStream_t s)
{
    if (!d->timing) return hipSuccess;
    return hipEventRecord(d->spans[d->spans_used++].b, s);
}

static inline dim3 flood_grid(const ldpc_decoder *d, unsigned blocks, unsigned tiles, int32_t *tiles_first, bool linked = false)
{
    const bool want = d->tune_tiles_first == 1 || (d->tune_tiles_first == 0 && linked);
    *tiles_first = (blocks <= 65535u && want) ? 1 : 0;
    return *tiles_first ? dim3(tiles, blocks) : dim3(blocks, tiles);
}

template <int V> int run_flooding(ldpc_decoder *d, const float *llr_dev, int64_t frames,
                                  uint8_t *out_dev, int64_t out_bytes, int32_t *iters_dev,
                                  hipStream_t s, int start_round = 1);

template <int V> int enqueue_check_phase(ldpc_decoder *d, hipStream_t s, int tiles, int64_t frames, int it, int max_iter,
                                         bool fat, const ldpc::TailRef &tr)
{
    using namespace ldpc;
    const int64_t msz = d->msg_size;
    for (auto &rc : d->row_classes) {
        if (!rc.linked) continue;
        HIP_TRY(span_begin(d, s, 4, rc.degree,
                           (2 * msz * rc.degree * rc.count + msz * 5 * rc.linked + 2 * msz * d->extra_edges) * frames,
                           msz * ((int64_t)rc.degree * rc.count + rc.linked +
                                  ((int64_t)rc.degree * rc.count - 2 * rc.linked) +
                                  (it < max_iter ? 2 * rc.linked : 0) + 2 * d->extra_edges) * frames));
        CheckArgs a{d->Q.p, d->R.p, rc.e0.p, d->done.p, d->E, rc.count, 1, rc.degree, d->ms_scale, tr};
        a.ms_offset = d->ms_offset;
        a.qpos = d->qpos.p;
        LinkArgs lk{rc.link_col.p, rc.link_pos.p, d->chan.p, d->Q.p, d->hard.p, d->N,
                    (it < max_iter) ? 1 : 0, d->tap_iter ? 1 : 0, d->extra_e0.p, d->extra_deg.p, d->n_extra, 0,
                    rc.n_big, rc.small_rows};
        a.rows_per_wave = d->link_rpw;
        const int variant = (d->tune_link_narrow == 2 && !d->link_half_fn[rc.degree]) ? 1 : d->tune_link_narrow;
        const int waves = link_chunk_count(d->link_rpw, rc.n_big, rc.small_rows, rc.count) * (variant == 1 ? V : variant == 2 ? V / 2 : 1);
        lk.link_blocks = (waves + kWavesPerBlock - 1) / kWavesPerBlock;
        const dim3 grid = flood_grid(d, lk.link_blocks + (d->n_extra + kWavesPerBlock - 1) / kWavesPerBlock, tiles, &a.tiles_first, true);
        (variant == 2 ? d->link_half_fn : variant == 1 ? (d->tune_link_deep ? d->link_deep_fn : d->link_narrow_fn) : d->link_fn)
            [rc.degree]<<<grid, kBlock, 0, s>>>(a, lk);
        HIP_TRY(span_end(d, s));
    }
    for (auto &g : d->check_groups) {
        int64_t edges = 0;
        for (int i : g.members) edges += (int64_t)d->row_classes[i].degree * d->row_classes[i].count;
        HIP_TRY(span_begin(d, s, 5, g.hi, 2 * msz * edges * frames, -1, g.lo));
        CheckArgs a{d->Q.p, d->R.p, nullptr, d->done.p, d->E, 0, (d->tune_rpw ? d->tune_rpw : 2) * (fat ? kIdleFat : 1), 0, d->ms_scale, tr};
        a.ms_offset = d->ms_offset;
        a.qpos = d->qpos.p;
        if (it == 1 && d->first_round_from_chan) { a.first_chan = d->chan.p; a.edge_col = d->edge_col.p; a.N = d->N; }
        const dim3 grid = flood_grid(d, fat ? g.blocks_fat : g.blocks, tiles, &a.tiles_first);
        d->check_group_fn[g.bucket]<<<grid, kBlock, 0, s>>>(a, fat ? g.table_fat.p : g.table.p, (int)g.members.size());
        HIP_TRY(span_end(d, s));
    }
    for (int ci : d->check_solo) {
        RowClass &rc = d->row_classes[ci];
        HIP_TRY(span_begin(d, s, 0, rc.degree, 2 * msz * rc.degree * rc.count * frames));
        CheckArgs a{d->Q.p, d->R.p, rc.e0.p, d->done.p, d->E, rc.count, 1, rc.degree, d->ms_scale, tr};
        a.ms_offset = d->ms_offset;
        a.qpos = d->qpos.p;
        if (it == 1 && d->first_round_from_chan) { a.first_chan = d->chan.p; a.edge_col = d->edge_col.p; a.N = d->N; }
        const int slotk = rc.degree <= d->max_check_unrolled ? rc.degree : 0;
        const bool narrow = slotk && (!d->tune_check_wide || rc.degree > kMaxUnrolledDegree);
        const int rpw = (d->tune_rpw ? d->tune_rpw : (narrow ? 2 : 1)) * (fat ? kIdleFat : 1);
        a.rows_per_wave = rpw;
        const int waves = ((rc.count + rpw - 1) / rpw) * (narrow ? V : 1);
        const dim3 grid = flood_grid(d, (waves + kWavesPerBlock - 1) / kWavesPerBlock, tiles, &a.tiles_first);
        (narrow ? d->check_fn : d->check_fn_wide)[slotk]<<<grid, kBlock, 0, s>>>(a);
        HIP_TRY(span_end(d, s));
    }
    return LDPC_OK;
}

template <int V> int enqueue_var_phase(ldpc_decoder *d, hipStream_t s, int tiles, int64_t frames, int it, int max_iter,
                                       bool fat, const ldpc::TailRef &tr)
{
    using namespace ldpc;
    const int64_t msz = d->msg_size;
    const int wq = (it < max_iter) ? 1 : 0;
    for (auto &g : d->var_groups) {
        int64_t units = 0;
        for (int i : g.members) units += (int64_t)((wq ? 2 : 1) * d->col_classes[i].degree + 1) * d->col_classes[i].count;
        HIP_TRY(span_begin(d, s, 6, g.hi, msz * units * frames, -1, g.lo));
        VarArgs a{d->R.p, d->Q.p, d->chan.p, d->hard.p, d->done.p, nullptr, nullptr,
                  d->E, d->N, 0, (d->tune_cpw ? d->tune_cpw : 1) * (fat ? kIdleFat : 1), wq, 0, tr};
        const dim3 grid = flood_grid(d, fat ? g.blocks_fat : g.blocks, tiles, &a.tiles_first);
        d->var_group_fn[g.bucket]<<<grid, kBlock, 0, s>>>(a, fat ? g.table_fat.p : g.table.p, (int)g.members.size());
        HIP_TRY(span_end(d, s));
    }
    for (int ci : d->var_solo) {
        ColClass &cc = d->col_classes[ci];
        HIP_TRY(span_begin(d, s, 1, cc.degree, msz * ((wq ? 2 : 1) * cc.degree + 1) * cc.count * frames));
        VarArgs a{d->R.p, d->Q.p, d->chan.p, d->hard.p, d->done.p, cc.col.p, cc.edge.p,
                  d->E, d->N, cc.count, 1, wq, cc.degree, tr};
        const int cpw = (d->tune_cpw ? d->tune_cpw : 1) * (fat ? kIdleFat : 1);
        a.cols_per_wave = cpw;
        a.q_base = cc.q_base;
        const int slotk = cc.degree <= kMaxUnrolledDegree ? cc.degree : 0;
        const int waves = (cc.count + cpw - 1) / cpw;
        const dim3 grid = flood_grid(d, (waves + kWavesPerBlock - 1) / kWavesPerBlock, tiles, &a.tiles_first);
        d->var_fn[slotk]<<<grid, kBlock, 0, s>>>(a);
        HIP_TRY(span_end(d, s));
    }
    return LDPC_OK;
}

template <int V> int compact_and_finish(ldpc_decoder *d, int64_t frames, int count, int it, hipStream_t s)
{
    using namespace ldpc;
    ldpc_decoder *c = d->child;
    while (c->child && count <= c->child->cfg.max_batch) c = c->child;
    const int cv = c->V, cf = 64 * cv;
    const unsigned ct = (unsigned)((count + cf - 1) / cf);
    const unsigned cg = ct * (unsigned)cv;
    if (cg > (unsigned)kBackWords) return fail(LDPC_ERR_STATE, "hand-over of %d frames: more than %d mask words per column", count, kBackWords);
    HIP_TRY(hipMemsetAsync(d->active.p, 0, sizeof(int32_t), s));
    compact_list_kernel<V><<<(unsigned)((frames + kBlock - 1) / kBlock), kBlock, 0, s>>>(d->done.p, frames, d->cmap.p,
                                                                                         d->active.p, d->child_capacity);
    const dim3 ge((unsigned)((d->E + kWavesPerBlock - 1) / kWavesPerBlock), cg);
    const dim3 gn((unsigned)((d->N + kWavesPerBlock - 1) / kWavesPerBlock), cg);
    const bool rowwise = count >= 128;
    const int ptiles = (int)((frames + 64 * V - 1) / (64 * V));
    if (d->msg_size == 2) {
        if (rowwise) {
            compact_gather_rows_kernel<V, _Float16><<<(unsigned)((d->E + gather_rows_per_block<_Float16>() - 1) / gather_rows_per_block<_Float16>()), kBlock, 0, s>>>((const _Float16 *)d->Q.p, (_Float16 *)c->Q.p, d->cmap.p, count, d->E, ptiles, cf, d->qpos.p, c->qpos.p);
            compact_gather_rows_kernel<V, _Float16><<<(unsigned)((d->N + gather_rows_per_block<_Float16>() - 1) / gather_rows_per_block<_Float16>()), kBlock, 0, s>>>((const _Float16 *)d->chan.p, (_Float16 *)c->chan.p, d->cmap.p, count, d->N, ptiles, cf);
        } else {
            compact_gather_kernel<V, _Float16><<<ge, kBlock, 0, s>>>((const _Float16 *)d->Q.p, (_Float16 *)c->Q.p, d->cmap.p, count, d->E, cf, d->qpos.p, c->qpos.p);
            compact_gather_kernel<V, _Float16><<<gn, kBlock, 0, s>>>((const _Float16 *)d->chan.p, (_Float16 *)c->chan.p, d->cmap.p, count, d->N, cf);
        }
    } else {
        if (rowwise) {
            compact_gather_rows_kernel<V, float><<<(unsigned)((d->E + gather_rows_per_block<float>() - 1) / gather_rows_per_block<float>()), kBlock, 0, s>>>((const float *)d->Q.p, (float *)c->Q.p, d->cmap.p, count, d->E, ptiles, cf, d->qpos.p, c->qpos.p);
            compact_gather_rows_kernel<V, float><<<(unsigned)((d->N + gather_rows_per_block<float>() - 1) / gather_rows_per_block<float>()), kBlock, 0, s>>>((const float *)d->chan.p, (float *)c->chan.p, d->cmap.p, count, d->N, ptiles, cf);
        } else {
            compact_gather_kernel<V, float><<<ge, kBlock, 0, s>>>((const float *)d->Q.p, (float *)c->Q.p, d->cmap.p, count, d->E, cf, d->qpos.p, c->qpos.p);
            compact_gather_kernel<V, float><<<gn, kBlock, 0, s>>>((const float *)d->chan.p, (float *)c->chan.p, d->cmap.p, count, d->N, cf);
        }
    }
    HIP_TRY(hipMemsetAsync(c->hard.p, 0, (size_t)ct * d->N * cv * sizeof(uint64_t), s));
    if (d->cfg.algo == LDPC_ALGO_SP) {
        if (ptiles * V <= kGatherParentWords && count <= 2 * kCompactCapacity)
            compact_hard_lds_kernel<V><<<(unsigned)((d->N + 63) / 64), kBlock, 0, s>>>(d->hard.p, c->hard.p, d->cmap.p, count, d->N, cv, ptiles, (int)cg);
        else
            compact_hard_kernel<V><<<gn, kBlock, 0, s>>>(d->hard.p, c->hard.p, d->cmap.p, count, d->N, cv);
    }
    compact_child_state_kernel<0><<<ct, 64, 0, s>>>(c->done.p, c->iters.p, count, d->cfg.max_iter, cv);
    HIP_TRY(hipGetLastError());
    c->timing = false;
    c->tap_iter = 0;
    const int rc = cv == 1 ? run_flooding<1>(c, nullptr, count, nullptr, 0, nullptr, s, it + 1)
                           : cv == 2 ? run_flooding<2>(c, nullptr, count, nullptr, 0, nullptr, s, it + 1)
                                     : run_flooding<4>(c, nullptr, count, nullptr, 0, nullptr, s, it + 1);
    if (rc) return rc;
    d->handed_to = c;
    HIP_TRY(hipMemsetAsync(d->cmoved.p, 0, d->cmoved.n * sizeof(unsigned long long), s));
    compact_inverse_kernel<V><<<(unsigned)((count + 255) / 256), 256, 0, s>>>(d->cmap.p, count, d->cinv.p, d->cmoved.p, cv);
    compact_hard_back_kernel<V><<<dim3((unsigned)((d->N + kBlock - 1) / kBlock), (unsigned)ptiles), kBlock, 0, s>>>(
        d->hard.p, c->hard.p, d->cinv.p, d->cmoved.p, d->N, cv, (int)cg);
    compact_finish_kernel<V><<<(unsigned)((count + 63) / 64), 64, 0, s>>>(d->done.p, d->iters.p, c->done.p, c->iters.p, d->cmap.p, count, cv);
    HIP_TRY(hipGetLastError());
    return LDPC_OK;
}

template <int V> int run_flooding(ldpc_decoder *d, const float *llr_dev, int64_t frames,
                                  uint8_t *out_dev, int64_t out_bytes, int32_t *iters_dev,
                                  hipStream_t s, int start_round)
{
    using namespace ldpc;
    const int F = 64 * V;
    const int tiles = (int)((frames + F - 1) / F);
    const int64_t msz = d->msg_size;
    const int max_iter = d->cfg.max_iter;
    const int rounds = d->tap_iter ? std::min(d->tap_iter, max_iter) : max_iter;
    const bool freeze = d->cfg.early_term != 0;
    const size_t slot = (size_t)d->TA * V;

    const bool resume = start_round > 1;
    HIP_TRY(hipMemsetAsync(d->failw.p, 0, d->failw.n * sizeof(uint64_t), s));
    HIP_TRY(hipMemsetAsync(d->summary.p, 0, 4 * sizeof(int32_t), s));
    d->handed_to = nullptr;
    if (!resume && d->summary_pending) {
        if (hipEventQuery(d->ev_summary) == hipSuccess) {
            d->summary_pending = false;
            d->idle_after = (d->h_summary[0] > 0 && d->h_summary[0] < max_iter) ? d->h_summary[0] + 1 : 0;
        } else {
            (void)hipGetLastError();
        }
    }
    const int idle_after = (freeze && !resume && !d->tap_iter && d->cfg.poll_interval == 0) ? d->idle_after : 0;
    const bool use_tail = d->tail_enabled && freeze && !resume && !d->tap_iter && tiles >= 4 * d->TO;
    const TailRef tr{use_tail ? d->tail_state.p : nullptr, d->T, d->TO};
    TailArgs ta{};
    if (use_tail) {
        HIP_TRY(hipMemsetAsync(d->tail_state.p, 0, 4 * sizeof(int32_t), s));
        HIP_TRY(hipMemsetAsync(d->running.p, 0, d->running.n * sizeof(int32_t), s));
        ta = TailArgs{d->tail_state.p, d->tail_map.p, d->running.p, d->done.p, d->iters.p, d->Q.p, d->chan.p, d->hard.p,
                      d->E, frames, d->N, tiles, d->T, d->TO * F, std::min(d->compact_threshold, d->TO * F), 0, max_iter};
    }

    bool q_less = d->cfg.algo == LDPC_ALGO_MS && !resume && !d->tap_iter && max_iter > 1 && d->n_extra == 0;
    for (auto &rc : d->row_classes) if (rc.linked) q_less = false;
    for (int ci : d->check_solo) if (d->row_classes[ci].degree > d->max_check_unrolled) q_less = false;
    d->first_round_from_chan = q_less;
    if (!resume) {
        HIP_TRY(span_begin(d, s, 3));
        InitArgs a{llr_dev, d->chan.p, q_less ? nullptr : d->Q.p, d->hard.p, d->col_ptr.p, d->col_qedge.p,
                   d->E, frames, d->N, d->cfg.llr_scale};
        dim3 grid((d->N + kInitCols - 1) / kInitCols, tiles);
        d->init_fn<<<grid, kBlock, 0, s>>>(a);
        StateArgs st{d->done.p, nullptr, d->iters.p, nullptr, frames, 0, max_iter, freeze ? 1 : 0};
        state_kernel<V><<<use_tail ? d->TA : tiles, 64, 0, s>>>(st);
        HIP_TRY(span_end(d, s));
    }

    int launched = start_round - 1;
    bool poll_dense = false;
    for (int it = start_round; it <= rounds; ++it) {
        const bool fat = idle_after > 0 && it > idle_after;
        {
            const int rcp = enqueue_check_phase<V>(d, s, tiles, frames, it, max_iter, fat, tr);
            if (rcp) return rcp;
        }
        {
            const int rcv = enqueue_var_phase<V>(d, s, tiles, frames, it, max_iter, fat, tr);
            if (rcv) return rcv;
        }
        launched = it;
        if (freeze || it == rounds) {
            HIP_TRY(span_begin(d, s, 3));
            uint64_t *fw = d->failw.p + (size_t)it * slot;
            const int rbk = (d->M + kBlock - 1) / kBlock;
            SyndromeArgs sa{d->row_ptr.p, d->edge_col.p, d->hard.p, fw, d->done.p, d->M, d->N,
                            d->tune_syn_xcd ? tiles : 0, rbk, tr};
            dim3 sgrid = d->tune_syn_xcd ? dim3(8 * rbk * ((tiles + 7) / 8)) : dim3(rbk, tiles);
            syndrome_kernel<V><<<sgrid, kBlock, 0, s>>>(sa);
            StateArgs st{d->done.p, fw, d->iters.p, nullptr, frames, it, max_iter, 1, tr, use_tail ? d->running.p : nullptr,
                         d->summary.p + 2};
            const bool poll = freeze && it < rounds && d->cfg.poll_interval > 0 && !d->suppress_poll &&
                              ((it % d->cfg.poll_interval) == 0 || poll_dense);
            if (poll) {
                HIP_TRY(hipMemsetAsync(d->active.p, 0, sizeof(int32_t), s));
                st.active = d->active.p;
            }
            state_kernel<V><<<tiles, 64, 0, s>>>(st);
            if (use_tail && it < rounds) {
                ta.iter = it;
                const unsigned tg = (unsigned)std::min<int64_t>(1024, d->E + 2 * (int64_t)d->N);
                if (d->msg_size == 2) tail_gather_kernel<V, _Float16><<<tg, kBlock, 0, s>>>(ta);
                else tail_gather_kernel<V, float><<<tg, kBlock, 0, s>>>(ta);
            }
            HIP_TRY(span_end(d, s));
            if (poll) {
                HIP_TRY(hipMemcpyAsync(d->h_active, d->active.p, sizeof(int32_t),
                                       hipMemcpyDeviceToHost, s));
                HIP_TRY(hipStreamSynchronize(s));
                const int running = *d->h_active;
                if (running == 0) break;
                if ((int64_t)running * 10 <= frames * 9 && d->child && tiles > 1 &&
                    (double)d->E * (double)frames * 4.0 * (double)msz > 1.5e9) poll_dense = true;
                if (d->child && running <= d->compact_threshold && (int64_t)running * 4 <= frames && tiles > 1 && !d->tap_iter) {
                    const int rc = compact_and_finish<V>(d, frames, running, it, s);
                    if (rc) return rc;
                    launched = d->handed_to->last_iterations;
                    break;
                }
            }
        }
    }
    d->last_iterations = launched;
    d->last_tiles = tiles;
    if (resume) return LDPC_OK;

    HIP_TRY(span_begin(d, s, 3));
    if (use_tail) tail_scatter_kernel<V><<<2048, kBlock, 0, s>>>(ta);
    {
        PackArgs pa{d->hard.p, out_dev, d->iters.p, iters_dev, frames, out_bytes, d->N, d->cfg.K,
                    d->cfg.pack_mode};
        const bool pack = (out_dev || iters_dev) && frames;
        if (d->cfg.pack_mode == LDPC_PACK_BYTES) {
            if (pack) pack_kernel<V><<<pack_grid<V>(d->cfg.K, tiles), kBlock, 0, s>>>(pa);
        } else {
            const int64_t n = std::max<int64_t>(out_bytes, frames);
            dim3 grid((unsigned)((n + kBlock - 1) / kBlock));
            if (pack) pack_kernel<V><<<grid, kBlock, 0, s>>>(pa);
        }
        summary_kernel<V><<<(unsigned)((frames + 255) / 256), 256, 0, s>>>(
            d->iters.p, d->done.p, d->failw.p, frames, 1, d->summary.p);
        if (!d->is_child && d->cfg.poll_interval == 0 && freeze && !d->summary_pending) {
            HIP_TRY(hipMemcpyAsync(d->h_summary, d->summary.p, 2 * sizeof(int32_t), hipMemcpyDeviceToHost, s));
            HIP_TRY(hipEventRecord(d->ev_summary, s));
            d->summary_pending = true;
        }
    }
    HIP_TRY(span_end(d, s));
    HIP_TRY(hipGetLastError());
    return LDPC_OK;
}

int build_classes(ldpc_decoder *d, const ldpc_graph *g)
{
    std::map<int, std::vector<int32_t>> rows_by_deg, cols_by_deg, rowids_by_deg;
    for (int32_t m = 0; m < g->M; ++m) {
        const int deg = g->row_ptr[m + 1] - g->row_ptr[m];
        if (deg > 0) { rows_by_deg[deg].push_back(g->row_ptr[m]); rowids_by_deg[deg].push_back(m); }
    }
    std::vector<char> fused_col((size_t)g->N, 0);
    d->row_classes.resize(rows_by_deg.size());
    size_t i = 0;
    for (auto &kv : rows_by_deg) {
        RowClass &rc = d->row_classes[i++];
        rc.degree = kv.first;
        rc.count = (int)kv.second.size();
        rc.h_e0 = kv.second;
        HIP_TRY(rc.e0.upload(kv.second));
        const std::vector<int32_t> &ids = rowids_by_deg[kv.first];
        const int rpw = d->link_rpw;
        if (rpw >= 2 && rc.degree >= 2 && rc.degree <= ldpc::kMaxUnrolledDegree) {
            rc.n_big = (rc.count + rpw - 1) / rpw;
            rc.small_rows = rpw;
            const int small = std::max(2, rpw / 4);
            const bool forced = ldpc::tune_forced_on(d->tune_link_guided);
            if ((d->T >= 4 || forced) && small < rpw && !ldpc::tune_forced_off(d->tune_link_guided)) {
                const int64_t last_generation = (int64_t)d->cus * 16 / d->T;
                int64_t big = (int64_t)rc.n_big - last_generation;
                if (big <= 0 && forced) big = rc.n_big - std::max(1, rc.n_big / 3);
                if (big > 0) { rc.n_big = (int)big; rc.small_rows = small; }
            }
            std::vector<char> chunk_end((size_t)rc.count, 0);
            for (int c = 0, nc = ldpc::link_chunk_count(rpw, rc.n_big, rc.small_rows, rc.count); c < nc; ++c) {
                int rb, re;
                ldpc::link_chunk_rows(c, rpw, rc.n_big, rc.small_rows, rc.count, &rb, &re);
                if (re > rb) chunk_end[(size_t)re - 1] = 1;
            }
            std::vector<int32_t> lcol((size_t)rc.count, -1), lpos((size_t)rc.count, 0);
            for (int idx = 0; idx + 1 < rc.count; ++idx) {
                if (chunk_end[idx]) continue;
                const int32_t m = ids[idx], m2 = ids[idx + 1];
                for (int32_t p = g->row_ptr[m]; p < g->row_ptr[m + 1]; ++p) {
                    const int32_t c = g->cols[p];
                    if (g->col_ptr[c + 1] - g->col_ptr[c] != 2 || fused_col[c]) continue;
                    const int32_t ea = g->col_edge[g->col_ptr[c]], eb = g->col_edge[g->col_ptr[c] + 1];
                    if (ea != p || g->rows[eb] != m2) continue;
                    lcol[idx] = c;
                    lpos[idx] = (p - g->row_ptr[m]) | ((eb - g->row_ptr[m2]) << 8);
                    fused_col[c] = 1;
                    ++rc.linked;
                    break;
                }
            }
            if (rc.linked * 4 >= rc.count) {
                HIP_TRY(rc.link_col.upload(lcol));
                HIP_TRY(rc.link_pos.upload(lpos));
            } else {
                for (int idx = 0; idx < rc.count; ++idx)
                    if (lcol[idx] >= 0) fused_col[lcol[idx]] = 0;
                rc.linked = 0;
            }
        }
    }
    for (int32_t n = 0; n < g->N; ++n) {
        const int deg = g->col_ptr[n + 1] - g->col_ptr[n];
        if (!fused_col[n]) cols_by_deg[deg].push_back(n);
    }
    d->col_classes.resize(cols_by_deg.size());
    i = 0;
    for (auto &kv : cols_by_deg) {
        ColClass &cc = d->col_classes[i++];
        cc.degree = kv.first;
        cc.count = (int)kv.second.size();
        std::vector<int32_t> edges;
        edges.reserve((size_t)cc.count * std::max(cc.degree, 1));
        for (int32_t n : kv.second)
            for (int32_t p = g->col_ptr[n]; p < g->col_ptr[n + 1]; ++p) edges.push_back(g->col_edge[p]);
        if (edges.empty()) edges.push_back(0);
        HIP_TRY(cc.col.upload(kv.second));
        HIP_TRY(cc.edge.upload(edges));
    }
    {
        d->h_qpos.assign((size_t)g->E, -1);
        int64_t slot = 0;
        if (d->tune.q_order >= 0)
            for (ColClass &cc : d->col_classes) {
                cc.q_base = slot;
                const std::vector<int32_t> &members = cols_by_deg[cc.degree];
                for (size_t ci = 0; ci < members.size(); ++ci)
                    for (int k = 0; k < cc.degree; ++k)
                        d->h_qpos[(size_t)g->col_edge[(size_t)g->col_ptr[members[ci]] + k]] = (int32_t)(slot + (int64_t)k * cc.count + (int64_t)ci);
                slot += (int64_t)cc.degree * cc.count;
            }
        for (int64_t e = 0; e < g->E; ++e)
            if (d->h_qpos[(size_t)e] < 0) d->h_qpos[(size_t)e] = d->tune.q_order >= 0 ? (int32_t)slot++ : (int32_t)e;
        std::vector<int32_t> cq((size_t)g->E);
        for (int64_t p = 0; p < g->E; ++p) cq[(size_t)p] = d->h_qpos[(size_t)g->col_edge[(size_t)p]];
        HIP_TRY(d->qpos.upload(d->h_qpos));
        HIP_TRY(d->col_qedge.upload(cq));
    }
    return LDPC_OK;
}

int plan_launches(ldpc_decoder *d)
{
    using ldpc::GroupClass;
    const int V = d->V;
    const bool merge = ldpc::tune_pick(d->tune.merge, true) && !d->tune_check_wide;
    d->check_groups.clear(); d->var_groups.clear(); d->check_solo.clear(); d->var_solo.clear();
    d->n_extra = 0; d->extra_edges = 0;
    int linked_classes = 0;
    int64_t unlinked_rows = 0;
    for (auto &rc : d->row_classes) { if (rc.linked) ++linked_classes; else unlinked_rows += rc.count; }
    const bool as_extra = merge && linked_classes == 1 && unlinked_rows > 0 && unlinked_rows <= 64;
    std::vector<int> cb[kCheckBuckets], vb[kVarBuckets];
    std::vector<int32_t> xe0, xdeg;
    for (int i = 0; i < (int)d->row_classes.size(); ++i) {
        RowClass &rc = d->row_classes[i];
        if (rc.linked) continue;
        if (as_extra) {
            for (int32_t e : rc.h_e0) { xe0.push_back(e); xdeg.push_back(rc.degree); d->extra_edges += rc.degree; }
            continue;
        }
        int b = -1;
        for (int k = 0; k < kCheckBuckets; ++k)
            if (rc.degree >= kCheckBucketLo[k] && rc.degree <= kCheckBucketHi[k] && rc.degree <= d->max_check_unrolled &&
                d->check_group_fn[k]) b = k;
        if (merge && b >= 0) cb[b].push_back(i); else d->check_solo.push_back(i);
    }
    if (as_extra) {
        d->n_extra = (int)xe0.size();
        HIP_TRY(d->extra_e0.upload(xe0));
        HIP_TRY(d->extra_deg.upload(xdeg));
    }
    for (int i = 0; i < (int)d->col_classes.size(); ++i) {
        const ColClass &cc = d->col_classes[i];
        int b = -1;
        for (int k = 0; k < kVarBuckets; ++k)
            if (cc.degree >= kVarBucketLo[k] && cc.degree <= kVarBucketHi[k] && d->var_group_fn[k]) b = k;
        if (merge && b >= 0) vb[b].push_back(i); else d->var_solo.push_back(i);
    }
    const int rpw = d->tune_rpw ? d->tune_rpw : 2, cpw = d->tune_cpw ? d->tune_cpw : 1;
    auto make = [&](std::vector<ClassGroup> &groups, std::vector<int> &solo, const std::vector<int> &members, int bucket,
                    int lo, int hi, bool rows) -> hipError_t {
        if (members.size() < 2) { for (int i : members) solo.push_back(i); return hipSuccess; }
        groups.emplace_back();
        ClassGroup &g = groups.back();
        g.bucket = bucket; g.lo = lo; g.hi = hi; g.members = members;
        std::vector<GroupClass> tab, tabf;
        constexpr int fatk = kIdleFat;
        for (int i : members) {
            GroupClass gc{};
            if (rows) {
                const RowClass &rc = d->row_classes[i];
                gc.degree = rc.degree; gc.count = rc.count; gc.ids = rc.e0.p; gc.edges = nullptr; gc.q_base = -1;
            } else {
                const ColClass &cc = d->col_classes[i];
                gc.degree = cc.degree; gc.count = cc.count; gc.ids = cc.col.p; gc.edges = cc.edge.p; gc.q_base = cc.q_base;
            }
            auto blocks_of = [&](int per_wave) {
                const int waves = ((gc.count + per_wave - 1) / per_wave) * (rows ? V / d->check_group_width : 1);
                return (waves + ldpc::kWavesPerBlock - 1) / ldpc::kWavesPerBlock;
            };
            gc.block_begin = g.blocks;
            tab.push_back(gc);
            g.blocks += blocks_of(rows ? rpw : cpw);
            gc.block_begin = g.blocks_fat;
            tabf.push_back(gc);
            g.blocks_fat += blocks_of((rows ? rpw : cpw) * fatk);
        }
        const hipError_t e = g.table.upload(tab);
        return e != hipSuccess ? e : g.table_fat.upload(tabf);
    };
    for (int k = 0; k < kCheckBuckets; ++k) HIP_TRY(make(d->check_groups, d->check_solo, cb[k], k, kCheckBucketLo[k], kCheckBucketHi[k], true));
    for (int k = 0; k < kVarBuckets; ++k) HIP_TRY(make(d->var_groups, d->var_solo, vb[k], k, kVarBucketLo[k], kVarBucketHi[k], false));
    return LDPC_OK;
}

int setup_flooding(ldpc_decoder *d, const ldpc_graph *g, size_t TF)
{
    const ldpc_decoder_config *cfg = &d->cfg;
    d->msg_size = cfg->msg_dtype == LDPC_MSG_F16 ? 2 : 4;
    HIP_TRY(d->chan.alloc(TF * d->N * d->msg_size));
    HIP_TRY(d->Q.alloc(TF * (size_t)d->E * d->msg_size));
    HIP_TRY(d->R.alloc(TF * (size_t)d->E * d->msg_size));
    int rc = build_classes(d, g);
    if (rc) return rc;
    ldpc::FloodFns fns;
    if (cfg->algo == LDPC_ALGO_SP) ldpc::fill_flood_sp(d->V, &fns);
    else if (d->ms_corr && cfg->msg_dtype == LDPC_MSG_F16) ldpc::fill_flood_msc16(d->V, &fns);
    else if (d->ms_corr) ldpc::fill_flood_msc(d->V, &fns);
    else if (cfg->msg_dtype == LDPC_MSG_F16) ldpc::fill_flood_ms16(d->V, &fns);
    else ldpc::fill_flood_ms(d->V, &fns);
    memcpy(d->check_fn, fns.check, sizeof fns.check);
    memcpy(d->check_fn_wide, fns.check_wide, sizeof fns.check_wide);
    memcpy(d->link_fn, fns.link, sizeof fns.link);
    memcpy(d->link_narrow_fn, fns.link_narrow, sizeof fns.link_narrow);
    memcpy(d->link_deep_fn, fns.link_deep, sizeof fns.link_deep);
    memcpy(d->link_half_fn, fns.link_half, sizeof fns.link_half);
    memcpy(d->var_fn, fns.var, sizeof fns.var);
    memcpy(d->check_group_fn, fns.check_group, sizeof fns.check_group);
    d->check_group_width = fns.check_group_width;
    memcpy(d->var_group_fn, fns.var_group, sizeof fns.var_group);
    d->init_fn = fns.init;
    d->max_check_unrolled = fns.max_check_unrolled;
    return plan_launches(d);
}

template <int V> int calibrate_link(ldpc_decoder *d)
{
    using namespace ldpc;
    RowClass *rcp = nullptr;
    for (auto &rc : d->row_classes) if (rc.linked) rcp = &rc;
    if (!rcp || !d->link_fn[rcp->degree] || !d->link_narrow_fn[rcp->degree]) return LDPC_OK;
    RowClass &rc = *rcp;
    const int tiles = d->T;
    hipStream_t s = d->stream;
    HIP_TRY(hipMemsetAsync(d->Q.p, 0, d->Q.n, s));
    HIP_TRY(hipMemsetAsync(d->chan.p, 0, d->chan.n, s));
    HIP_TRY(hipMemsetAsync(d->done.p, 0, d->done.n * sizeof(uint64_t), s));
    hipEvent_t ev[2] = {nullptr, nullptr};
    HIP_TRY(hipEventCreate(&ev[0]));
    HIP_TRY(hipEventCreate(&ev[1]));
    float best[3] = {1e30f, 1e30f, 1e30f};
    const int candidates = d->link_half_fn[rc.degree] ? 3 : 2;
    hipError_t err = hipSuccess;
    for (int rep = 0; rep < 4 && err == hipSuccess; ++rep) {
        for (int nar = 0; nar < candidates && err == hipSuccess; ++nar) {
            CheckArgs a{d->Q.p, d->R.p, rc.e0.p, d->done.p, d->E, rc.count, d->link_rpw, rc.degree, d->ms_scale,
                        TailRef{nullptr, 0, 0}};
            a.ms_offset = d->ms_offset;
            a.qpos = d->qpos.p;
            LinkArgs lk{rc.link_col.p, rc.link_pos.p, d->chan.p, d->Q.p, d->hard.p, d->N, 1, 0, nullptr, nullptr, 0, 0,
                        rc.n_big, rc.small_rows};
            const int waves = link_chunk_count(d->link_rpw, rc.n_big, rc.small_rows, rc.count) * (nar == 1 ? V : nar == 2 ? V / 2 : 1);
            lk.link_blocks = (waves + kWavesPerBlock - 1) / kWavesPerBlock;
            const dim3 grid = flood_grid(d, lk.link_blocks, tiles, &a.tiles_first, true);
            err = hipEventRecord(ev[0], s);
            (nar == 2 ? d->link_half_fn : nar == 1 ? d->link_narrow_fn : d->link_fn)[rc.degree]<<<grid, kBlock, 0, s>>>(a, lk);
            if (err == hipSuccess) err = hipEventRecord(ev[1], s);
            if (err == hipSuccess) err = hipEventSynchronize(ev[1]);
            float ms = 0;
            if (err == hipSuccess) err = hipEventElapsedTime(&ms, ev[0], ev[1]);
            if (err == hipSuccess && rep > 0 && ms < best[nar]) best[nar] = ms;
        }
    }
    (void)hipEventDestroy(ev[0]);
    (void)hipEventDestroy(ev[1]);
    if (err != hipSuccess) return fail(LDPC_ERR_HIP, "link calibration: %s", hipGetErrorString(err));
    HIP_TRY(hipGetLastError());
    int pick = 0;
    for (int k = 0; k < candidates; ++k) { d->link_cal_ms[k] = best[k]; if (best[k] < best[pick]) pick = k; }
    d->tune_link_narrow = pick;
    d->link_calibrated = true;
    return LDPC_OK;
}

template <int V> int time_check_phase(ldpc_decoder *d, float *ms_out)
{
    hipStream_t s = d->stream;
    HIP_TRY(hipMemsetAsync(d->Q.p, 0, d->Q.n, s));
    HIP_TRY(hipMemsetAsync(d->chan.p, 0, d->chan.n, s));
    HIP_TRY(hipMemsetAsync(d->done.p, 0, d->done.n * sizeof(uint64_t), s));
    hipEvent_t ev[2] = {nullptr, nullptr};
    HIP_TRY(hipEventCreate(&ev[0]));
    HIP_TRY(hipEventCreate(&ev[1]));
    float best = 1e30f;
    hipError_t err = hipSuccess;
    int rc = LDPC_OK;
    for (int rep = 0; rep < 4 && err == hipSuccess && rc == LDPC_OK; ++rep) {
        err = hipEventRecord(ev[0], s);
        rc = enqueue_check_phase<V>(d, s, d->T, (int64_t)d->T * d->F, 1, d->cfg.max_iter, false, ldpc::TailRef{nullptr, 0, 0});
        if (rc == LDPC_OK)
            rc = enqueue_var_phase<V>(d, s, d->T, (int64_t)d->T * d->F, 1, d->cfg.max_iter, false, ldpc::TailRef{nullptr, 0, 0});
        if (err == hipSuccess) err = hipEventRecord(ev[1], s);
        if (err == hipSuccess) err = hipEventSynchronize(ev[1]);
        float ms = 0;
        if (err == hipSuccess) err = hipEventElapsedTime(&ms, ev[0], ev[1]);
        if (err == hipSuccess && rep > 0 && ms < best) best = ms;
    }
    (void)hipEventDestroy(ev[0]);
    (void)hipEventDestroy(ev[1]);
    if (rc) return rc;
    if (err != hipSuccess) return fail(LDPC_ERR_HIP, "placement search: %s", hipGetErrorString(err));
    *ms_out = best;
    return LDPC_OK;
}

template <int V> int placement_search(ldpc_decoder *d, size_t TF)
{
    const size_t bq = TF * (size_t)d->E * d->msg_size, bc = TF * d->N * d->msg_size;
    const int want = d->tune.place == 0 ? (2 * bq + bc >= ((size_t)256 << 20) ? 6 : 1) : d->tune.place;
    if (want <= 1) return LDPC_OK;
    float best_ms = 0.0f;
    int rc = time_check_phase<V>(d, &best_ms);
    if (rc) return rc;
    std::vector<DevBuf<uint8_t>> held;
    d->place_ms[0] = best_ms;
    d->place_candidates = 1;
    d->place_kept = 0;
    float lo = best_ms, hi = best_ms;
    for (int stage = 0; stage < 2; ++stage) {
        DevBuf<uint8_t> &arr = stage == 0 ? d->R : d->Q;
        for (int c = 1; c < want; ++c) {
            if (lo < 0.91f * hi && best_ms <= lo && d->place_candidates >= 4) break;
            size_t free_b = 0, total_b = 0;
            if (hipMemGetInfo(&free_b, &total_b) != hipSuccess || free_b < 2 * bq + ((size_t)2 << 30)) break;
            DevBuf<uint8_t> cand, spacer;
            const size_t period = (size_t)16 << 30;
            if (c == 1 && arr.n < period && free_b > period + 2 * bq + ((size_t)2 << 30)) {
                if (spacer.alloc(period - arr.n) != hipSuccess) (void)hipGetLastError();
            }
            if (cand.alloc(arr.n) != hipSuccess) { (void)hipGetLastError(); break; }
            spacer.release();
            std::swap(arr, cand);
            float ms = 0.0f;
            rc = time_check_phase<V>(d, &ms);
            if (rc) return rc;
            if (d->place_candidates < 16) d->place_ms[d->place_candidates] = ms;
            lo = std::min(lo, ms); hi = std::max(hi, ms);
            if (ms < best_ms) {
                best_ms = ms;
                d->place_kept = d->place_candidates;
            } else {
                std::swap(arr, cand);
            }
            ++d->place_candidates;
            held.push_back(std::move(cand));
        }
    }
    return LDPC_OK;
}

}


static thread_local int t_child_depth = 0;

extern "C" {

int ldpc_abi_version(void) { return LDPC_HIP_ABI_VERSION; }

const char *ldpc_last_error(void) { return g_err.c_str(); }

int ldpc_device_count(int *count)
{
    if (!count) return fail(LDPC_ERR_ARG, "count is NULL");
    *count = 0;
    int n = 0;
    hipError_t e = hipGetDeviceCount(&n);
    if (e != hipSuccess) return fail(LDPC_ERR_HIP, "hipGetDeviceCount: %s", hipGetErrorString(e));
    *count = n;
    return LDPC_OK;
}

int64_t ldpc_out_bytes(int32_t K, int64_t frames, int32_t pack_mode)
{
    if (frames <= 0 || K <= 0) return 0;
    if (pack_mode == LDPC_PACK_BYTES) return (frames - 1) * (int64_t)K / 8 + K / 8;
    return (frames * (int64_t)K + 7) / 8;
}

int ldpc_graph_create(const int32_t *rows, const int32_t *cols, int64_t E, int32_t M, int32_t N,
                      ldpc_graph **out)
{
    if (!out) return fail(LDPC_ERR_ARG, "out is NULL");
    *out = nullptr;
    if (!rows || !cols) return fail(LDPC_ERR_ARG, "rows/cols is NULL");
    if (M <= 0 || N <= 0 || E <= 0) return fail(LDPC_ERR_ARG, "M, N, E must be positive");
    if (E > 0x7fffffffLL) return fail(LDPC_ERR_ARG, "E does not fit int32 edge ids");
    for (int64_t e = 0; e < E; ++e) {
        if (rows[e] < 0 || rows[e] >= M || cols[e] < 0 || cols[e] >= N)
            return fail(LDPC_ERR_ARG, "edge %lld = (%d, %d) outside %d x %d", (long long)e, rows[e],
                        cols[e], M, N);
        if (e && (rows[e] < rows[e - 1] || (rows[e] == rows[e - 1] && cols[e] <= cols[e - 1])))
            return fail(LDPC_ERR_ARG, "edges must be in strictly ascending row-major order (edge %lld)",
                        (long long)e);
    }
    ldpc_graph *g = new (std::nothrow) ldpc_graph;
    if (!g) return fail(LDPC_ERR_NOMEM, "out of memory");
    g->M = M; g->N = N; g->E = E;
    g->rows.assign(rows, rows + E);
    g->cols.assign(cols, cols + E);
    g->row_ptr.assign((size_t)M + 1, 0);
    g->col_ptr.assign((size_t)N + 1, 0);
    for (int64_t e = 0; e < E; ++e) { ++g->row_ptr[rows[e] + 1]; ++g->col_ptr[cols[e] + 1]; }
    for (int32_t m = 0; m < M; ++m) {
        g->max_row_deg = std::max(g->max_row_deg, g->row_ptr[m + 1]);
        g->row_ptr[m + 1] += g->row_ptr[m];
    }
    for (int32_t n = 0; n < N; ++n) {
        g->max_col_deg = std::max(g->max_col_deg, g->col_ptr[n + 1]);
        g->col_ptr[n + 1] += g->col_ptr[n];
    }
    g->col_edge.assign((size_t)E, 0);
    std::vector<int32_t> fill(g->col_ptr.begin(), g->col_ptr.end() - 1);
    for (int64_t e = 0; e < E; ++e) g->col_edge[fill[cols[e]]++] = (int32_t)e;
    *out = g;
    return LDPC_OK;
}

int ldpc_graph_destroy(ldpc_graph *g)
{
    delete g;
    return LDPC_OK;
}

int ldpc_graph_info(const ldpc_graph *g, int32_t *M, int32_t *N, int64_t *E, int32_t *max_row_deg,
                    int32_t *max_col_deg)
{
    if (!g) return fail(LDPC_ERR_ARG, "graph is NULL");
    if (M) *M = g->M;
    if (N) *N = g->N;
    if (E) *E = g->E;
    if (max_row_deg) *max_row_deg = g->max_row_deg;
    if (max_col_deg) *max_col_deg = g->max_col_deg;
    return LDPC_OK;
}

void ldpc_decoder_config_init(ldpc_decoder_config *cfg)
{
    if (!cfg) return;
    memset(cfg, 0, sizeof *cfg);
    cfg->struct_size = sizeof *cfg;
    cfg->max_batch = 1;
    cfg->algo = LDPC_ALGO_SP;
    cfg->msg_dtype = LDPC_MSG_F32;
    cfg->max_iter = 40;
    cfg->llr_scale = 8.0f;
    cfg->early_term = 1;
    cfg->pack_mode = LDPC_PACK_BYTES;
}

static int config_in(const ldpc_decoder_config *cfg, ldpc_decoder_config *full)
{
    constexpr size_t kSizeBeforeMsCorr = offsetof(ldpc_decoder_config, ms_scale);
    if (cfg->struct_size != sizeof(ldpc_decoder_config) && cfg->struct_size != kSizeBeforeMsCorr)
        return fail(LDPC_ERR_ARG, "config struct_size %u is neither %zu nor %zu (ABI mismatch)", cfg->struct_size,
                    sizeof(ldpc_decoder_config), kSizeBeforeMsCorr);
    memset(full, 0, sizeof *full);
    memcpy(full, cfg, cfg->struct_size);
    full->struct_size = sizeof *full;
    return LDPC_OK;
}

int ldpc_decoder_create(const ldpc_graph *g, const ldpc_decoder_config *cfg_in, ldpc_decoder **out)
{
    if (!out) return fail(LDPC_ERR_ARG, "out is NULL");
    *out = nullptr;
    if (!g || !cfg_in) return fail(LDPC_ERR_ARG, "graph/config is NULL");
    ldpc_decoder_config cfg_full;
    if (int rc = config_in(cfg_in, &cfg_full)) return rc;
    const ldpc_decoder_config *cfg = &cfg_full;
    if (cfg->K <= 0 || cfg->K > g->N) return fail(LDPC_ERR_ARG, "K=%d out of range", cfg->K);
    if (cfg->max_batch <= 0) return fail(LDPC_ERR_ARG, "max_batch must be positive");
    if (cfg->max_iter <= 0 || cfg->max_iter > 100000) return fail(LDPC_ERR_ARG, "max_iter out of range");
    if (cfg->algo != LDPC_ALGO_SP && cfg->algo != LDPC_ALGO_MS && cfg->algo != LDPC_ALGO_LAYERED &&
        cfg->algo != LDPC_ALGO_MS_FUSED && cfg->algo != LDPC_ALGO_LAYERED_HOST)
        return fail(LDPC_ERR_ARG, "unknown algo %d", cfg->algo);
    if (!(cfg->ms_scale >= 0.0f && cfg->ms_scale <= 1.0f))
        return fail(LDPC_ERR_ARG, "ms_scale must be 0 (off) or in (0, 1]");
    if (!(cfg->ms_offset >= 0.0f && cfg->ms_offset < 1000.0f))
        return fail(LDPC_ERR_ARG, "ms_offset must be 0 (off) or in (0, 1000)");
    const bool ms_corr = cfg->ms_scale != 0.0f || cfg->ms_offset != 0.0f;
    if (ms_corr && cfg->algo != LDPC_ALGO_MS && cfg->algo != LDPC_ALGO_LAYERED)
        return fail(LDPC_ERR_UNSUPPORTED, "ms_scale / ms_offset apply to LDPC_ALGO_MS and LDPC_ALGO_LAYERED only "
                    "(SP has no minimum to correct; MS_FUSED and LAYERED_HOST reproduce reference kernels)");
    if (cfg->algo == LDPC_ALGO_LAYERED_HOST) {
        for (int32_t m = 1; m < g->M; ++m)
            if (g->row_ptr[m + 1] - g->row_ptr[m] != g->row_ptr[1] - g->row_ptr[0])
                return fail(LDPC_ERR_UNSUPPORTED, "LAYERED_HOST follows the reference's host-layered path, which sizes its "
                            "layers correctly only when every row of H has the same weight (MyLdpc.cpp:907,958)");
        if (g->max_row_deg > ldpc::kMaxUnrolledLayerDegree)
            return fail(LDPC_ERR_UNSUPPORTED, "LAYERED_HOST: row weight %d > %d", g->max_row_deg, ldpc::kMaxUnrolledLayerDegree);
    }
    if (cfg->pack_mode != LDPC_PACK_BYTES && cfg->pack_mode != LDPC_PACK_BITS)
        return fail(LDPC_ERR_ARG, "unknown pack_mode %d", cfg->pack_mode);
    if (cfg->frames_per_lane != 0 && cfg->frames_per_lane != 1 && cfg->frames_per_lane != 2 &&
        cfg->frames_per_lane != 4)
        return fail(LDPC_ERR_ARG, "frames_per_lane must be 0, 1, 2 or 4");
    if (cfg->msg_dtype != LDPC_MSG_F32 && cfg->msg_dtype != LDPC_MSG_F16)
        return fail(LDPC_ERR_ARG, "unknown msg_dtype %d", cfg->msg_dtype);
    if (cfg->msg_dtype == LDPC_MSG_F16 && cfg->algo != LDPC_ALGO_MS)
        return fail(LDPC_ERR_UNSUPPORTED, "fp16 messages are built for flooding min-sum only "
                    "(the probability-domain SP needs fp32 range; layered: not yet)");
    if (!ldpc::tune_valid(*cfg)) return fail(LDPC_ERR_ARG, "tuning / streams config fields out of range");

    int ndev = 0;
    HIP_TRY(hipGetDeviceCount(&ndev));
    if (cfg->device < 0 || cfg->device >= ndev)
        return fail(LDPC_ERR_HIP, "device %d not present (%d HIP devices)", cfg->device, ndev);
    HIP_TRY(hipSetDevice(cfg->device));

    ldpc_decoder *d = new (std::nothrow) ldpc_decoder;
    if (!d) return fail(LDPC_ERR_NOMEM, "out of memory");
    std::unique_ptr<ldpc_decoder> guard(d);
    d->cfg = *cfg;
    d->ms_corr = ms_corr;
    d->ms_scale = cfg->ms_scale != 0.0f ? cfg->ms_scale : 1.0f;
    d->ms_offset = cfg->ms_offset;
    d->M = g->M; d->N = g->N; d->E = g->E;
    d->h_col_ptr = g->col_ptr; d->h_col_edge = g->col_edge; d->h_rows = g->rows; d->h_cols = g->cols;
    const ldpc::Tune tune = d->tune = ldpc::tune_from_config(*cfg);
    d->tune_rpw = tune.rows_per_wave;
// ... 1036 lines not shown
```

Measured before the change: 1022 Mbit/s.

## Compute first-round check messages from channel values for all algorithms

Extends the first-iteration shortcut, where check nodes read channel values directly instead of Q, to sum-product and to linked, generic and extra-row kernels. For sum-product the channel value is turned into the probability-domain difference message on the fly. The init kernel then no longer writes the full Q array, which removes one E-sized write pass and one gather read per decode. The cost is many more kernel template instantiations and extra dispatch tables.

```diff
diff --git a/myldpccppapi_amd/csrc/flood_kernels.hpp b/myldpccppapi_amd/csrc/flood_kernels.hpp
--- a/myldpccppapi_amd/csrc/flood_kernels.hpp
+++ b/myldpccppapi_amd/csrc/flood_kernels.hpp
@@ -164,6 +164,19 @@
     return tiles_first ? GridPos{(int)blockIdx.x, (int)blockIdx.y} : GridPos{(int)blockIdx.y, (int)blockIdx.x};
 }
 
+template <int ALGO> __device__ __forceinline__ float first_msg(float c)
+{
+    if (ALGO == kAlgoSP) return c / (1.0f + c) - 1.0f / (1.0f + c);
+    return c;
+}
+template <int ALGO, int D, int V> __device__ __forceinline__ void first_msgs(float (&x)[D][V])
+{
+#pragma unroll
+    for (int k = 0; k < D; ++k)
+#pragma unroll
+        for (int v = 0; v < V; ++v) x[k][v] = first_msg<ALGO>(x[k][v]);
+}
+
 template <int D, int V>
 __device__ __forceinline__ void check_sp(const float (&x)[D][V], float (&out)[D][V])
 {
@@ -224,7 +237,7 @@
 
 __device__ __forceinline__ MsCorr ms_corr_of(const CheckArgs &a) { return MsCorr{a.ms_scale, a.ms_offset}; }
 
-template <int ALGO, int D, int V, int W, typename T>
+template <int ALGO, int D, int V, int W, typename T, bool FIRST = false>
 __global__ __launch_bounds__(kBlock) void check_kernel(const CheckArgs a)
 {
     constexpr size_t F = 64 * V;
@@ -241,14 +254,15 @@
     const T *Qu = static_cast<const T *>(a.Q) + (size_t)tile * (size_t)a.E * F;
     T *Rt = static_cast<T *>(a.R) + (size_t)tile * (size_t)a.E * F + lane_off;
 
-    const T *Ct = (ALGO != kAlgoSP && a.first_chan)
+    const T *Ct = ((FIRST || ALGO != kAlgoSP) && a.first_chan)
                       ? static_cast<const T *>(a.first_chan) + (size_t)tile * (size_t)a.N * F + lane_off : nullptr;
     for (int r = r_begin; r < r_end; ++r) {
         const int e0 = a.cls_e0[r];
         float x[D][W], out[D][W];
-        if (ALGO != kAlgoSP && Ct) {
+        if (FIRST || (ALGO != kAlgoSP && Ct)) {
 #pragma unroll
             for (int k = 0; k < D; ++k) vload<W>(x[k], Ct + (size_t)a.edge_col[e0 + k] * F);
+            first_msgs<ALGO, D, W>(x);
         } else {
             int sl[D];
             row_slots<D>(a.qpos, e0, lane, sl);
@@ -263,9 +277,19 @@
 
 template <int ALGO, int V, typename T>
 __device__ __forceinline__ void check_row_generic(const T *Qu, unsigned lane_off, T *Rt, int e0, int D,
-                                                  const int32_t *__restrict__ qpos, const MsCorr &c)
+                                                  const int32_t *__restrict__ qpos, const MsCorr &c,
+                                                  const T *Ct = nullptr, const int32_t *__restrict__ edge_col = nullptr)
 {
     constexpr size_t F = 64 * V;
+    auto load_msg = [&](float (&xj)[V], int j) {
+        if (Ct) {
+            vload<V>(xj, Ct + (size_t)__builtin_amdgcn_readfirstlane(edge_col[e0 + j]) * F);
+#pragma unroll
+            for (int v = 0; v < V; ++v) xj[v] = first_msg<ALGO>(xj[v]);
+        } else {
+            vload<V>(xj, Qu + (size_t)edge_slot(qpos, e0 + j) * F + lane_off);
+        }
+    };
     if (ALGO != kAlgoSP) {
         float m1[V], m2[V];
         int idx[V];
@@ -274,7 +298,7 @@
         for (int v = 0; v < V; ++v) { m1[v] = 1000.0f; m2[v] = 1000.0f; idx[v] = -1; par[v] = 0; }
         for (int j = 0; j < D; ++j) {
             float xj[V];
-            vload<V>(xj, Qu + (size_t)edge_slot(qpos, e0 + j) * F + lane_off);
+            load_msg(xj, j);
 #pragma unroll
             for (int v = 0; v < V; ++v) {
                 const float m = __builtin_fabsf(xj[v]);
@@ -289,7 +313,7 @@
         }
         for (int k = 0; k < D; ++k) {
             float xk[V], o[V];
-            vload<V>(xk, Qu + (size_t)edge_slot(qpos, e0 + k) * F + lane_off);
+            load_msg(xk, k);
 #pragma unroll
             for (int v = 0; v < V; ++v) {
                 const float b = (k == idx[v]) ? m2[v] : m1[v];
@@ -308,7 +332,7 @@
         for (int j = 0; j < D; ++j) {
             if (j == k) continue;
             float xj[V];
-            vload<V>(xj, Qu + (size_t)edge_slot(qpos, e0 + j) * F + lane_off);
+            load_msg(xj, j);
 #pragma unroll
             for (int v = 0; v < V; ++v) p[v] *= xj[v];
         }
@@ -318,7 +342,7 @@
     }
 }
 
-template <int ALGO, int V, typename T>
+template <int ALGO, int V, typename T, bool FIRST = false>
 __global__ __launch_bounds__(kBlock) void check_kernel_generic(const CheckArgs a)
 {
     constexpr size_t F = 64 * V;
@@ -331,7 +355,9 @@
     const int r_end = min(r_begin + a.rows_per_wave, a.n_rows);
     const T *Qu = static_cast<const T *>(a.Q) + (size_t)tile * (size_t)a.E * F;
     T *Rt = static_cast<T *>(a.R) + (size_t)tile * (size_t)a.E * F + (size_t)lane * V;
-    for (int r = r_begin; r < r_end; ++r) check_row_generic<ALGO, V, T>(Qu, (unsigned)lane * V, Rt, a.cls_e0[r], a.degree, a.qpos, ms_corr_of(a));
+    const T *Ct = FIRST ? static_cast<const T *>(a.first_chan) + (size_t)tile * (size_t)a.N * F + (size_t)lane * V : nullptr;
+    for (int r = r_begin; r < r_end; ++r)
+        check_row_generic<ALGO, V, T>(Qu, (unsigned)lane * V, Rt, a.cls_e0[r], a.degree, a.qpos, ms_corr_of(a), Ct, a.edge_col);
 }
 
 struct GroupClass {
@@ -344,7 +370,7 @@
     int64_t q_base;
 };
 
-template <int ALGO, int D, int V, int W, typename T>
+template <int ALGO, int D, int V, int W, typename T, bool FIRST>
 __device__ __forceinline__ void check_rows(const T *Qu, unsigned lane_off, T *Rt, const int32_t *__restrict__ e0s, int r_begin, int r_end,
                                            const T *Ct, const int32_t *__restrict__ edge_col,
                                            const int32_t *__restrict__ qpos, const MsCorr &c)
@@ -354,9 +380,10 @@
     for (int r = r_begin; r < r_end; ++r) {
         const int e0 = e0s[r];
         float x[D][W], out[D][W];
-        if (ALGO != kAlgoSP && Ct) {
+        if (FIRST || (ALGO != kAlgoSP && Ct)) {
 #pragma unroll
             for (int k = 0; k < D; ++k) vload<W>(x[k], Ct + (size_t)edge_col[e0 + k] * F);
+            first_msgs<ALGO, D, W>(x);
         } else {
             int sl[D];
             row_slots<D>(qpos, e0, lane, sl);
@@ -369,23 +396,23 @@
     }
 }
 
-template <int ALGO, int V, typename T, int D, int DLO, int W = 1> struct CheckDispatch {
+template <int ALGO, int V, typename T, int D, int DLO, int W, bool FIRST> struct CheckDispatch {
     static __device__ __forceinline__ void run(int deg, const T *Qu, unsigned lane_off, T *Rt, const int32_t *e0s, int rb, int re,
                                                const T *Ct, const int32_t *edge_col, const int32_t *qpos, const MsCorr &c)
     {
-        if (deg == D) check_rows<ALGO, D, V, W, T>(Qu, lane_off, Rt, e0s, rb, re, Ct, edge_col, qpos, c);
-        else CheckDispatch<ALGO, V, T, D - 1, DLO, W>::run(deg, Qu, lane_off, Rt, e0s, rb, re, Ct, edge_col, qpos, c);
+        if (deg == D) check_rows<ALGO, D, V, W, T, FIRST>(Qu, lane_off, Rt, e0s, rb, re, Ct, edge_col, qpos, c);
+        else CheckDispatch<ALGO, V, T, D - 1, DLO, W, FIRST>::run(deg, Qu, lane_off, Rt, e0s, rb, re, Ct, edge_col, qpos, c);
     }
 };
-template <int ALGO, int V, typename T, int DLO, int W> struct CheckDispatch<ALGO, V, T, DLO, DLO, W> {
+template <int ALGO, int V, typename T, int DLO, int W, bool FIRST> struct CheckDispatch<ALGO, V, T, DLO, DLO, W, FIRST> {
     static __device__ __forceinline__ void run(int, const T *Qu, unsigned lane_off, T *Rt, const int32_t *e0s, int rb, int re,
                                                const T *Ct, const int32_t *edge_col, const int32_t *qpos, const MsCorr &c)
     {
-        check_rows<ALGO, DLO, V, W, T>(Qu, lane_off, Rt, e0s, rb, re, Ct, edge_col, qpos, c);
+        check_rows<ALGO, DLO, V, W, T, FIRST>(Qu, lane_off, Rt, e0s, rb, re, Ct, edge_col, qpos, c);
     }
 };
 
-template <int ALGO, int V, typename T, int DLO, int DHI, int W = 1>
+template <int ALGO, int V, typename T, int DLO, int DHI, int W = 1, bool FIRST = false>
 __global__ __launch_bounds__(kBlock) void check_group_kernel(const CheckArgs a, const GroupClass *__restrict__ cls, int n_classes)
 {
     constexpr size_t F = 64 * V;
@@ -403,9 +430,9 @@
     const unsigned lane_off = (unsigned)sub * 64 * W + (unsigned)lane * W;
     const T *Qu = static_cast<const T *>(a.Q) + (size_t)tile * (size_t)a.E * F;
     T *Rt = static_cast<T *>(a.R) + (size_t)tile * (size_t)a.E * F + lane_off;
-    const T *Ct = (ALGO != kAlgoSP && a.first_chan)
+    const T *Ct = ((FIRST || ALGO != kAlgoSP) && a.first_chan)
                       ? static_cast<const T *>(a.first_chan) + (size_t)tile * (size_t)a.N * F + lane_off : nullptr;
-    CheckDispatch<ALGO, V, T, DHI, DLO, W>::run(cls[c].degree, Qu, lane_off, Rt, cls[c].ids, r_begin, r_end, Ct, a.edge_col, a.qpos, ms_corr_of(a));
+    CheckDispatch<ALGO, V, T, DHI, DLO, W, FIRST>::run(cls[c].degree, Qu, lane_off, Rt, cls[c].ids, r_begin, r_end, Ct, a.edge_col, a.qpos, ms_corr_of(a));
 }
 
 struct SyndromeArgs {
@@ -552,7 +579,7 @@
     return n_big + (rest > 0 ? (rest + small_rows - 1) / small_rows : 0);
 }
 
-template <int ALGO, int V, typename T>
+template <int ALGO, int V, typename T, bool FIRST>
 __device__ __forceinline__ void link_extra_rows(const CheckArgs &a, const LinkArgs &g, int tile, int block)
 {
     constexpr size_t F = 64 * V;
@@ -561,7 +588,8 @@
     if (w >= g.n_extra) return;
     const T *Qu = static_cast<const T *>(a.Q) + (size_t)tile * (size_t)a.E * F;
     T *Rt = static_cast<T *>(a.R) + (size_t)tile * (size_t)a.E * F + (size_t)lane * V;
-    check_row_generic<ALGO, V, T>(Qu, (unsigned)lane * V, Rt, g.extra_e0[w], g.extra_deg[w], a.qpos, ms_corr_of(a));
+    const T *Ct = FIRST ? static_cast<const T *>(a.first_chan) + (size_t)tile * (size_t)a.N * F + (size_t)lane * V : nullptr;
+    check_row_generic<ALGO, V, T>(Qu, (unsigned)lane * V, Rt, g.extra_e0[w], g.extra_deg[w], a.qpos, ms_corr_of(a), Ct, a.edge_col);
 }
 
 #ifdef LDPC_LINK_WIDE_WAVES
@@ -569,7 +597,7 @@
 #else
 #define LDPC_LINK_WIDE_ATTR
 #endif
-template <int ALGO, int D, int V, typename T>
+template <int ALGO, int D, int V, typename T, bool FIRST = false>
 __global__ __launch_bounds__(kBlock) LDPC_LINK_WIDE_ATTR void check_link_kernel(const CheckArgs a, const LinkArgs g)
 {
     constexpr size_t F = 64 * V;
@@ -577,7 +605,7 @@
     const GridPos gp = grid_pos(a.tiles_first);
     const int tile = tile_select<V>(a.tail, a.done, gp.row);
     if (tile < 0) return;
-    if (gp.block >= g.link_blocks) { link_extra_rows<ALGO, V, T>(a, g, tile, gp.block); return; }
+    if (gp.block >= g.link_blocks) { link_extra_rows<ALGO, V, T, FIRST>(a, g, tile, gp.block); return; }
     const int wave = gp.block * kWavesPerBlock + wave_id_in_block();
     int r_begin, r_end;
     link_chunk_rows(wave, a.rows_per_wave, g.n_big, g.small_rows, a.n_rows, &r_begin, &r_end);
@@ -604,7 +632,10 @@
     if (r_begin < r_end) {
         row_slots<D>(a.qpos, a.cls_e0[r_begin], lane, qc);
 #pragma unroll
-        for (int k = 0; k < D; ++k) vload<V>(x[k], Qt + (size_t)qc[k] * F + lane_q);
+        for (int k = 0; k < D; ++k) {
+            if (FIRST) vload<V>(x[k], chan_t + (size_t)a.edge_col[a.cls_e0[r_begin] + k] * F);
+            else vload<V>(x[k], Qt + (size_t)qc[k] * F + lane_q);
+        }
     }
     for (int r = r_begin; r < r_end; ++r) {
         const int e0 = a.cls_e0[r];
@@ -621,10 +652,14 @@
             for (int v = 0; v < V; ++v) old_w[v] = hard_t[(size_t)pend_col * V + v];
         }
         float out[D][V];
+        if (FIRST) first_msgs<ALGO, D, V>(x);
         if (ALGO == kAlgoSP) check_sp<D, V>(x, out); else if (ALGO == kAlgoMS) check_ms<D, V>(x, out); else check_ms<D, V, true, T>(x, out, ms_corr_of(a));
         if (r + 1 < r_end) {
 #pragma unroll
-            for (int k = 0; k < D; ++k) vload<V>(x[k], Qt + (size_t)qn[k] * F + lane_q);
+            for (int k = 0; k < D; ++k) {
+                if (FIRST) vload<V>(x[k], chan_t + (size_t)a.edge_col[a.cls_e0[r + 1] + k] * F);
+                else vload<V>(x[k], Qt + (size_t)qn[k] * F + lane_q);
+            }
         }
 #pragma unroll
         for (int k = 0; k < D; ++k)
@@ -713,7 +748,7 @@
     return x;
 }
 
-template <int ALGO, int D, int V, typename T, int W = 1>
+template <int ALGO, int D, int V, typename T, int W = 1, bool FIRST = false>
 __global__ __launch_bounds__(kBlock) void check_link_narrow_kernel(const CheckArgs a, const LinkArgs g)
 {
     constexpr size_t F = 64 * V;
@@ -723,7 +758,7 @@
     const GridPos gp = grid_pos(a.tiles_first);
     const int tile = tile_select<V>(a.tail, a.done, gp.row);
     if (tile < 0) return;
-    if (gp.block >= g.link_blocks) { link_extra_rows<ALGO, V, T>(a, g, tile, gp.block); return; }
+    if (gp.block >= g.link_blocks) { link_extra_rows<ALGO, V, T, FIRST>(a, g, tile, gp.block); return; }
     const int wave = gp.block * kWavesPerBlock + wave_id_in_block();
     const int sub = wave % SUBS;
     int r_begin, r_end;
@@ -756,7 +791,10 @@
     if (r_begin < r_end) {
         row_slots<D>(a.qpos, a.cls_e0[r_begin], lane, qc);
 #pragma unroll
-        for (int k = 0; k < D; ++k) vload<W>(x[k], Qt + (size_t)qc[k] * F + lane_q);
+        for (int k = 0; k < D; ++k) {
+            if (FIRST) vload<W>(x[k], chan_t + (size_t)a.edge_col[a.cls_e0[r_begin] + k] * F);
+            else vload<W>(x[k], Qt + (size_t)qc[k] * F + lane_q);
+        }
     }
     for (int r = r_begin; r < r_end; ++r) {
         const int e0 = a.cls_e0[r];
@@ -775,10 +813,14 @@
             for (int w = 0; w < W; ++w) old_mine[w] = load_field(pend_col, (W * lane + w) % V);
         }
         float out[D][W];
+        if (FIRST) first_msgs<ALGO, D, W>(x);
         if (ALGO == kAlgoSP) check_sp<D, W>(x, out); else if (ALGO == kAlgoMS) check_ms<D, W>(x, out); else check_ms<D, W, true, T>(x, out, ms_corr_of(a));
         if (r + 1 < r_end) {
 #pragma unroll
-            for (int k = 0; k < D; ++k) vload<W>(x[k], Qt + (size_t)qn[k] * F + lane_q);
+            for (int k = 0; k < D; ++k) {
+                if (FIRST) vload<W>(x[k], chan_t + (size_t)a.edge_col[a.cls_e0[r + 1] + k] * F);
+                else vload<W>(x[k], Qt + (size_t)qn[k] * F + lane_q);
+            }
         }
 #pragma unroll
         for (int k = 0; k < D; ++k)
@@ -854,7 +896,7 @@
     }
 }
 
-template <int ALGO, int D, int V, typename T>
+template <int ALGO, int D, int V, typename T, bool FIRST = false>
 __global__ __launch_bounds__(kBlock) void check_link_narrow2_kernel(const CheckArgs a, const LinkArgs g)
 {
     constexpr size_t F = 64 * V;
@@ -863,7 +905,7 @@
     const GridPos gp = grid_pos(a.tiles_first);
     const int tile = tile_select<V>(a.tail, a.done, gp.row);
     if (tile < 0) return;
-    if (gp.block >= g.link_blocks) { link_extra_rows<ALGO, V, T>(a, g, tile, gp.block); return; }
+    if (gp.block >= g.link_blocks) { link_extra_rows<ALGO, V, T, FIRST>(a, g, tile, gp.block); return; }
     const int wave = gp.block * kWavesPerBlock + wave_id_in_block();
     const int sub = wave % V;
     int r_begin, r_end;
@@ -891,7 +933,12 @@
     auto load_row = [&](float (&dst)[D], int r) {
         const int e = a.cls_e0[r];
 #pragma unroll
-        for (int k = 0; k < D; ++k) { float t[1]; vload<1>(t, Qt + (size_t)edge_slot(a.qpos, e + k) * F); dst[k] = t[0]; }
+        for (int k = 0; k < D; ++k) {
+            float t[1];
+            if (FIRST) vload<1>(t, chan_t + (size_t)__builtin_amdgcn_readfirstlane(a.edge_col[e + k]) * F);
+            else vload<1>(t, Qt + (size_t)edge_slot(a.qpos, e + k) * F);
+            dst[k] = t[0];
+        }
     };
     if (r_begin < r_end) load_row(b0, r_begin);
     if (r_begin + 1 < r_end) load_row(b1, r_begin + 1);
@@ -910,7 +957,7 @@
         if (r + 2 < r_end) load_row(pre, r + 2);
         float xx[D][1], out[D][1];
 #pragma unroll
-        for (int k = 0; k < D; ++k) xx[k][0] = x[k];
+        for (int k = 0; k < D; ++k) xx[k][0] = FIRST ? first_msg<ALGO>(x[k]) : x[k];
         if (ALGO == kAlgoSP) check_sp<D, 1>(xx, out); else if (ALGO == kAlgoMS) check_ms<D, 1>(xx, out); else check_ms<D, 1, true, T>(xx, out, ms_corr_of(a));
 #pragma unroll
         for (int k = 0; k < D; ++k)
diff --git a/myldpccppapi_amd/csrc/flood_tables.hpp b/myldpccppapi_amd/csrc/flood_tables.hpp
--- a/myldpccppapi_amd/csrc/flood_tables.hpp
+++ b/myldpccppapi_amd/csrc/flood_tables.hpp
@@ -22,6 +22,10 @@
     LinkFn link_narrow[kMaxUnrolledDegree + 1] = {};
     LinkFn link_deep[kMaxUnrolledDegree + 1] = {};
     LinkFn link_half[kMaxUnrolledDegree + 1] = {};
+    LinkFn link_first[kMaxUnrolledDegree + 1] = {}, link_narrow_first[kMaxUnrolledDegree + 1] = {},
+           link_deep_first[kMaxUnrolledDegree + 1] = {}, link_half_first[kMaxUnrolledDegree + 1] = {};
+    CheckFn check_first[kMaxUnrolledCheckDegreeMS + 1] = {}, check_wide_first[kMaxUnrolledCheckDegreeMS + 1] = {};
+    CheckGroupFn check_group_first[kCheckBuckets] = {};
     VarFn var[kMaxUnrolledDegree + 1] = {};
     CheckGroupFn check_group[kCheckBuckets] = {};
     int check_group_width = 1;
diff --git a/myldpccppapi_amd/csrc/flood_tables_impl.hpp b/myldpccppapi_amd/csrc/flood_tables_impl.hpp
--- a/myldpccppapi_amd/csrc/flood_tables_impl.hpp
+++ b/myldpccppapi_amd/csrc/flood_tables_impl.hpp
@@ -33,31 +33,46 @@
     static void fill(CheckFn *, CheckFn *) {}
 };
 
-template <int ALGO, int V, typename T, int D> struct LinkHalf {
+template <int ALGO, int V, typename T, int D, bool FIRST> struct LinkHalf {
     static LinkFn get() { return nullptr; }
 };
-template <int ALGO, typename T, int D> struct LinkHalf<ALGO, 4, T, D> {
-    static LinkFn get() { return check_link_narrow_kernel<ALGO, D, 4, T, 2>; }
+template <int ALGO, typename T, int D, bool FIRST> struct LinkHalf<ALGO, 4, T, D, FIRST> {
+    static LinkFn get() { return check_link_narrow_kernel<ALGO, D, 4, T, 2, FIRST>; }
 };
-template <int ALGO, int V, typename T, int D> struct LinkTable {
+template <int ALGO, int V, typename T, int D, bool FIRST> struct LinkTable {
     static void fill(LinkFn *t, LinkFn *tn, LinkFn *td, LinkFn *th)
     {
-        t[D] = check_link_kernel<ALGO, D, V, T>;
-        tn[D] = check_link_narrow_kernel<ALGO, D, V, T>;
-        td[D] = check_link_narrow2_kernel<ALGO, D, V, T>;
-        th[D] = LinkHalf<ALGO, V, T, D>::get();
-        LinkTable<ALGO, V, T, D - 1>::fill(t, tn, td, th);
+        t[D] = check_link_kernel<ALGO, D, V, T, FIRST>;
+        tn[D] = check_link_narrow_kernel<ALGO, D, V, T, 1, FIRST>;
+        td[D] = check_link_narrow2_kernel<ALGO, D, V, T, FIRST>;
+        th[D] = LinkHalf<ALGO, V, T, D, FIRST>::get();
+        LinkTable<ALGO, V, T, D - 1, FIRST>::fill(t, tn, td, th);
     }
 };
-template <int ALGO, int V, typename T> struct LinkTable<ALGO, V, T, 1> {
+template <int ALGO, int V, typename T, bool FIRST> struct LinkTable<ALGO, V, T, 1, FIRST> {
     static void fill(LinkFn *, LinkFn *, LinkFn *, LinkFn *) {}
+};
+
+template <int ALGO, int V, typename T, int D> struct FirstTable {
+    static void fill(FloodFns *f)
+    {
+        if (ALGO == kAlgoSP) {
+            f->check_first[D] = check_kernel<ALGO, D, V, 1, T, (ALGO == kAlgoSP)>;
+            f->check_wide_first[D] = check_kernel<ALGO, D, V, V, T, (ALGO == kAlgoSP)>;
+        }
+        FirstTable<ALGO, V, T, D - 1>::fill(f);
+    }
+};
+template <int ALGO, int V, typename T> struct FirstTable<ALGO, V, T, 0> {
+    static void fill(FloodFns *f) { f->check_first[0] = f->check_wide_first[0] = check_kernel_generic<ALGO, V, T, true>; }
 };
 
 template <int ALGO, int V, typename T> void fill_v(FloodFns *f)
 {
     constexpr int DM = kMaxUnrolledDegree;
     FloodTable<ALGO, V, T, DM>::fill(f->check, f->check_wide, f->var);
-    LinkTable<ALGO, V, T, DM>::fill(f->link, f->link_narrow, f->link_deep, f->link_half);
+    LinkTable<ALGO, V, T, DM, false>::fill(f->link, f->link_narrow, f->link_deep, f->link_half);
+    LinkTable<ALGO, V, T, DM, true>::fill(f->link_first, f->link_narrow_first, f->link_deep_first, f->link_half_first);
     constexpr int GW = (sizeof(T) == 2 && V == 4) ? 2 : 1;
     f->check_group_width = GW;
     f->check_group[0] = check_group_kernel<ALGO, V, T, 1, 8, GW>;
@@ -74,6 +89,13 @@
         f->check_group[3] = check_group_kernel<ALGO, V, T, 25, 32, GW>;
         f->max_check_unrolled = kMaxUnrolledCheckDegreeMS;
     }
+    for (int d = 1; d <= kMaxUnrolledCheckDegreeMS; ++d) { f->check_first[d] = f->check[d]; f->check_wide_first[d] = f->check_wide[d]; }
+    for (int k = 0; k < kCheckBuckets; ++k) f->check_group_first[k] = f->check_group[k];
+    if (ALGO == kAlgoSP) {
+        f->check_group_first[0] = check_group_kernel<ALGO, V, T, 1, 8, GW, (ALGO == kAlgoSP)>;
+        f->check_group_first[1] = check_group_kernel<ALGO, V, T, 9, 16, GW, (ALGO == kAlgoSP)>;
+    }
+    FirstTable<ALGO, V, T, DM>::fill(f);
 }
 
 template <int ALGO, typename T> void fill(int V, FloodFns *f)
diff --git a/myldpccppapi_amd/csrc/ldpc_hip.hip b/myldpccppapi_amd/csrc/ldpc_hip.hip
--- a/myldpccppapi_amd/csrc/ldpc_hip.hip
+++ b/myldpccppapi_amd/csrc/ldpc_hip.hip
@@ -174,6 +174,8 @@
     std::vector<ClassGroup> check_groups, var_groups;
     std::vector<int> check_solo, var_solo;
     CheckGroupFn check_group_fn[kCheckBuckets] = {};
+    CheckGroupFn check_group_first_fn[kCheckBuckets] = {};
+    CheckFn check_first_fn[ldpc::kMaxUnrolledCheckDegreeMS + 1] = {}, check_wide_first_fn[ldpc::kMaxUnrolledCheckDegreeMS + 1] = {};
     int check_group_width = 1;
     VarGroupFn var_group_fn[kVarBuckets] = {};
     DevBuf<int32_t> extra_e0, extra_deg;
@@ -186,6 +188,7 @@
     LinkFn link_narrow_fn[ldpc::kMaxUnrolledDegree + 1] = {};
     LinkFn link_deep_fn[ldpc::kMaxUnrolledDegree + 1] = {};
     LinkFn link_half_fn[ldpc::kMaxUnrolledDegree + 1] = {};
+    LinkFn link_first_fn[4][ldpc::kMaxUnrolledDegree + 1] = {};
     int tune_link_deep = 0;
     ldpc::Tune tune;
     int tune_link_narrow = 1;
@@ -405,8 +408,11 @@
         const int waves = link_chunk_count(d->link_rpw, rc.n_big, rc.small_rows, rc.count) * (variant == 1 ? V : variant == 2 ? V / 2 : 1);
         lk.link_blocks = (waves + kWavesPerBlock - 1) / kWavesPerBlock;
         const dim3 grid = flood_grid(d, lk.link_blocks + (d->n_extra + kWavesPerBlock - 1) / kWavesPerBlock, tiles, &a.tiles_first, true);
-        (variant == 2 ? d->link_half_fn : variant == 1 ? (d->tune_link_deep ? d->link_deep_fn : d->link_narrow_fn) : d->link_fn)
-            [rc.degree]<<<grid, kBlock, 0, s>>>(a, lk);
+        const bool first = it == 1 && d->first_round_from_chan;
+        if (first) { a.first_chan = d->chan.p; a.edge_col = d->edge_col.p; a.N = d->N; }
+        const LinkFn *fns = variant == 2 ? d->link_half_fn : variant == 1 ? (d->tune_link_deep ? d->link_deep_fn : d->link_narrow_fn) : d->link_fn;
+        if (first) fns = d->link_first_fn[variant == 2 ? 3 : variant == 1 ? (d->tune_link_deep ? 2 : 1) : 0];
+        fns[rc.degree]<<<grid, kBlock, 0, s>>>(a, lk);
         HIP_TRY(span_end(d, s));
     }
     for (auto &g : d->check_groups) {
@@ -416,9 +422,10 @@
         CheckArgs a{d->Q.p, d->R.p, nullptr, d->done.p, d->E, 0, (d->tune_rpw ? d->tune_rpw : 2) * (fat ? kIdleFat : 1), 0, d->ms_scale, tr};
         a.ms_offset = d->ms_offset;
         a.qpos = d->qpos.p;
-        if (it == 1 && d->first_round_from_chan) { a.first_chan = d->chan.p; a.edge_col = d->edge_col.p; a.N = d->N; }
+        const bool first = it == 1 && d->first_round_from_chan;
+        if (first) { a.first_chan = d->chan.p; a.edge_col = d->edge_col.p; a.N = d->N; }
         const dim3 grid = flood_grid(d, fat ? g.blocks_fat : g.blocks, tiles, &a.tiles_first);
-        d->check_group_fn[g.bucket]<<<grid, kBlock, 0, s>>>(a, fat ? g.table_fat.p : g.table.p, (int)g.members.size());
+        (first ? d->check_group_first_fn : d->check_group_fn)[g.bucket]<<<grid, kBlock, 0, s>>>(a, fat ? g.table_fat.p : g.table.p, (int)g.members.size());
         HIP_TRY(span_end(d, s));
     }
     for (int ci : d->check_solo) {
@@ -427,14 +434,15 @@
         CheckArgs a{d->Q.p, d->R.p, rc.e0.p, d->done.p, d->E, rc.count, 1, rc.degree, d->ms_scale, tr};
         a.ms_offset = d->ms_offset;
         a.qpos = d->qpos.p;
-        if (it == 1 && d->first_round_from_chan) { a.first_chan = d->chan.p; a.edge_col = d->edge_col.p; a.N = d->N; }
+        const bool first = it == 1 && d->first_round_from_chan;
+        if (first) { a.first_chan = d->chan.p; a.edge_col = d->edge_col.p; a.N = d->N; }
         const int slotk = rc.degree <= d->max_check_unrolled ? rc.degree : 0;
         const bool narrow = slotk && (!d->tune_check_wide || rc.degree > kMaxUnrolledDegree);
         const int rpw = (d->tune_rpw ? d->tune_rpw : (narrow ? 2 : 1)) * (fat ? kIdleFat : 1);
         a.rows_per_wave = rpw;
         const int waves = ((rc.count + rpw - 1) / rpw) * (narrow ? V : 1);
         const dim3 grid = flood_grid(d, (waves + kWavesPerBlock - 1) / kWavesPerBlock, tiles, &a.tiles_first);
-        (narrow ? d->check_fn : d->check_fn_wide)[slotk]<<<grid, kBlock, 0, s>>>(a);
+        (first ? (narrow ? d->check_first_fn : d->check_wide_first_fn) : (narrow ? d->check_fn : d->check_fn_wide))[slotk]<<<grid, kBlock, 0, s>>>(a);
         HIP_TRY(span_end(d, s));
     }
     return LDPC_OK;
@@ -567,9 +575,7 @@
                       d->E, frames, d->N, tiles, d->T, d->TO * F, std::min(d->compact_threshold, d->TO * F), 0, max_iter};
     }
 
-    bool q_less = d->cfg.algo == LDPC_ALGO_MS && !resume && !d->tap_iter && max_iter > 1 && d->n_extra == 0;
-    for (auto &rc : d->row_classes) if (rc.linked) q_less = false;
-    for (int ci : d->check_solo) if (d->row_classes[ci].degree > d->max_check_unrolled) q_less = false;
+    const bool q_less = !resume && !d->tap_iter && max_iter > 1;
     d->first_round_from_chan = q_less;
     if (!resume) {
         HIP_TRY(span_begin(d, s, 3));
@@ -863,8 +869,15 @@
     memcpy(d->link_narrow_fn, fns.link_narrow, sizeof fns.link_narrow);
     memcpy(d->link_deep_fn, fns.link_deep, sizeof fns.link_deep);
     memcpy(d->link_half_fn, fns.link_half, sizeof fns.link_half);
+    memcpy(d->link_first_fn[0], fns.link_first, sizeof fns.link_first);
+    memcpy(d->link_first_fn[1], fns.link_narrow_first, sizeof fns.link_narrow_first);
+    memcpy(d->link_first_fn[2], fns.link_deep_first, sizeof fns.link_deep_first);
+    memcpy(d->link_first_fn[3], fns.link_half_first, sizeof fns.link_half_first);
     memcpy(d->var_fn, fns.var, sizeof fns.var);
     memcpy(d->check_group_fn, fns.check_group, sizeof fns.check_group);
+    memcpy(d->check_group_first_fn, fns.check_group_first, sizeof fns.check_group_first);
+    memcpy(d->check_first_fn, fns.check_first, sizeof fns.check_first);
+    memcpy(d->check_wide_first_fn, fns.check_wide_first, sizeof fns.check_wide_first);
     d->check_group_width = fns.check_group_width;
     memcpy(d->var_group_fn, fns.var_group, sizeof fns.var_group);
     d->init_fn = fns.init;
```

New measurement: 1007 Mbit/s. 0.985x the previous value.
